# DOGECOIN87/firedancer

Measured on AMD Instinct MI355X. Metric: verified ed25519 sigs/sec (node), higher is better.
Workload: dtype u32; 1 GPU; cfg2: 1000000 single-sig txns/GPU, msg U[180,220] B, 90% valid / 10% corrupted, device-resident batch, full verify + per-txn combine per step; parallelism=dp1 (independent per-GPU batches), queues=2

## Files before the change

firedancer_amd/_lib.py:

```python
import ctypes
import os

_HERE = os.path.dirname(os.path.abspath(__file__))
LIB_PATH = os.environ.get("FDGPU_LIB") or os.path.join(_HERE, "libfd_ed25519_gpu.so")
HEADER_PATH = os.path.join(os.path.dirname(_HERE), "include", "fd_ed25519_gpu.h")
SHRED_HEADER_PATH = os.path.join(os.path.dirname(_HERE), "include", "fd_shred_gpu.h")
POH_HEADER_PATH = os.path.join(os.path.dirname(_HERE), "include", "fd_poh_gpu.h")

_LIB = None


class FdgpuTxn(ctypes.Structure):
    _fields_ = [("msg_off", ctypes.c_uint32), ("msg_sz", ctypes.c_uint32),
                ("sig_off", ctypes.c_uint32), ("pub_off", ctypes.c_uint32),
                ("sig_cnt", ctypes.c_uint32)]


class FdgpuCfg(ctypes.Structure):
    _fields_ = [("max_txn", ctypes.c_uint64), ("max_sig", ctypes.c_uint64),
                ("max_arena", ctypes.c_uint64), ("ring_depth", ctypes.c_uint32),
                ("flags", ctypes.c_uint32)]


def lib():
    global _LIB
    if _LIB is not None:
        return _LIB
    if not os.path.exists(LIB_PATH):
        raise RuntimeError(f"firedancer_amd: engine library not built: {LIB_PATH} "
                           "(run `make -C firedancer_amd/csrc`)")
    L = ctypes.CDLL(LIB_PATH)
    c = ctypes
    vp, u8p = c.c_void_p, c.c_char_p
    L.fd_ed25519_verify.argtypes = [u8p, c.c_uint64, u8p, u8p, vp]
    L.fd_ed25519_verify.restype = c.c_int
    L.fd_ed25519_verify_batch_single_msg.argtypes = [u8p, c.c_uint64, u8p, u8p, vp, c.c_uint8]
    L.fd_ed25519_verify_batch_single_msg.restype = c.c_int
    L.fd_ed25519_strerror.argtypes = [c.c_int]
    L.fd_ed25519_strerror.restype = c.c_char_p
    L.fdgpu_engine_open.argtypes = [c.c_int, c.POINTER(FdgpuCfg)]
    L.fdgpu_engine_open.restype = vp
    L.fdgpu_engine_reserve.argtypes = [vp, c.c_uint64]
    L.fdgpu_engine_reserve.restype = c.c_int
    L.fdgpu_engine_close.argtypes = [vp]
    L.fdgpu_engine_close.restype = None
    L.fdgpu_last_error.argtypes = []
    L.fdgpu_last_error.restype = c.c_char_p
    L.fdgpu_device_count.argtypes = []
    L.fdgpu_device_count.restype = c.c_int
    L.fdgpu_kernel_path.argtypes = []
    L.fdgpu_kernel_path.restype = c.c_char_p
    L.fdgpu_build_info.argtypes = []
    L.fdgpu_build_info.restype = c.c_char_p
    L.fdgpu_submit.argtypes = [vp, vp, c.c_uint64, vp, c.c_uint64]
    L.fdgpu_submit.restype = c.c_int64
    L.fdgpu_poll.argtypes = [vp, c.c_int64, vp, c.c_int]
    L.fdgpu_poll.restype = c.c_int
    L.fdgpu_stage_acquire.argtypes = [vp, c.POINTER(c.c_uint64)]
    L.fdgpu_stage_acquire.restype = vp
    L.fdgpu_stage_submit.argtypes = [vp, c.c_uint64, vp, c.c_uint64]
    L.fdgpu_stage_submit.restype = c.c_int64
    L.fdgpu_poll_keep.argtypes = [vp, c.c_int64, vp, c.c_int]
    L.fdgpu_poll_keep.restype = c.c_int
    L.fdgpu_release.argtypes = [vp, c.c_int64]
    L.fdgpu_release.restype = c.c_int
    L.fdgpu_stage_cancel.argtypes = [vp]
    L.fdgpu_stage_cancel.restype = c.c_int
    L.fdgpu_host_register.argtypes = [vp, vp, c.c_uint64]
    L.fdgpu_host_register.restype = c.c_int
    L.fdgpu_host_unregister.argtypes = [vp, vp]
    L.fdgpu_host_unregister.restype = c.c_int
    L.fdgpu_verify_device.argtypes = [vp, vp, vp, c.c_uint64, vp, c.c_uint64, vp, vp, vp]
    L.fdgpu_verify_device.restype = c.c_int
    L.fdgpu_engine_info.argtypes = [vp, c.POINTER(c.c_uint32), c.POINTER(c.c_uint32), c.POINTER(c.c_uint64)]
    L.fdgpu_engine_info.restype = c.c_int
    L.fdgpu_debug_fe_ops.argtypes = [vp, vp, c.c_uint64, vp]
    L.fdgpu_debug_decode.argtypes = [vp, vp, c.c_uint64, c.c_int, vp]
    L.fdgpu_debug_sha512.argtypes = [vp, vp, c.c_uint64, vp, c.c_uint64, vp]
    L.fdgpu_debug_hram.argtypes = [vp, vp, c.c_uint64, vp, c.c_uint64, vp]
    L.fdgpu_debug_sc_reduce.argtypes = [vp, vp, c.c_uint64, vp]
    L.fdgpu_debug_hs_split.argtypes = [vp, vp, c.c_uint64, vp]
    L.fdgpu_debug_sig_codes.argtypes = [vp, vp, c.c_uint64, vp, c.c_uint64, vp]
    L.fdgpu_dev_batch_upload.argtypes = [vp, vp, c.c_uint64, vp, c.c_uint64]
    L.fdgpu_dev_batch_upload.restype = vp
    L.fdgpu_dev_batch_verify.argtypes = [vp, vp]
    L.fdgpu_dev_batch_verify.restype = c.c_int
    L.fdgpu_dev_batch_own_queue.argtypes = [vp, vp]
    L.fdgpu_dev_batch_own_queue.restype = c.c_int
    L.fdgpu_dev_batch_codes.argtypes = [vp, vp, vp, vp]
    L.fdgpu_dev_batch_codes.restype = c.c_int
    L.fdgpu_dev_batch_upload_frags.argtypes = [vp, vp, c.c_uint64, vp, c.c_uint64]
    L.fdgpu_dev_batch_upload_frags.restype = vp
    L.fdgpu_dev_batch_txns.argtypes = [vp, vp, vp, vp]
    L.fdgpu_dev_batch_txns.restype = c.c_int
    L.fdgpu_dev_batch_time2.argtypes = [vp, vp, c.c_int] + [c.POINTER(c.c_double)] * 4
    L.fdgpu_dev_batch_time2.restype = c.c_int
    L.fdgpu_dev_batch_free.argtypes = [vp, vp]
    L.fdgpu_dev_batch_free.restype = None
    L.fdgpu_dev_batch_sig_cnt.argtypes = [vp]
    L.fdgpu_dev_batch_sig_cnt.restype = c.c_uint64
    L.fdgpu_dev_batch_device_ptrs.argtypes = [vp] + [vp] * 6
    L.fdgpu_dev_batch_device_ptrs.restype = c.c_int
    L.fdgpu_dev_batch_time.argtypes = [vp, vp, c.c_int, c.POINTER(c.c_double), c.POINTER(c.c_double),
                                       c.POINTER(c.c_double)]
    L.fdgpu_dev_batch_time.restype = c.c_int
    L.fdgpu_sync.argtypes = [vp]
    L.fdgpu_sync.restype = c.c_int
    L.fdgpu_submit_frags.argtypes = [vp, vp, c.c_uint64, vp, c.c_uint64, c.c_uint64]
    L.fdgpu_submit_frags.restype = c.c_int64
    L.fdgpu_poll_frags.argtypes = [vp, c.c_int64, vp, vp, c.c_int]
    L.fdgpu_poll_frags.restype = c.c_int
    L.fdgpu_submit_frags_io.argtypes = [vp, vp, c.c_uint64, vp, c.c_uint64, c.c_uint64, vp, c.c_uint64]
    L.fdgpu_submit_frags_io.restype = c.c_int64
    L.fdgpu_poll_frags_io.argtypes = [vp, c.c_int64, vp, vp, vp, c.c_int]
    L.fdgpu_poll_frags_io.restype = c.c_int
    L.fdgpu_debug_submit_times.argtypes = [vp, c.c_uint64]
    L.fdgpu_debug_submit_times.restype = c.c_uint64
    L.fdgpu_debug_h2d_gbps.argtypes = [vp, vp, c.c_uint64, c.c_int]
    L.fdgpu_debug_h2d_gbps.restype = c.c_double
    L.fdgpu_frag_out_cap.argtypes = [c.c_uint32]
    L.fdgpu_frag_out_cap.restype = c.c_uint32
    L.fdgpu_ed25519_verify.argtypes = [u8p, c.c_uint64, u8p, u8p]
    L.fdgpu_ed25519_verify.restype = c.c_int
    L.fdgpu_ed25519_verify_batch_single_msg.argtypes = [u8p, c.c_uint64, u8p, u8p, c.c_uint8]
    L.fdgpu_ed25519_verify_batch_single_msg.restype = c.c_int
    L.fdgpu_sync_stats.argtypes = [c.POINTER(c.c_uint64)] * 3
    L.fdgpu_sync_stats.restype = None
    L.fdgpu_sync_errors.argtypes = []
    L.fdgpu_sync_errors.restype = c.c_uint64
    L.fdgpu_submit_shreds.argtypes = [vp, vp, c.c_uint64, vp, c.c_uint64, c.c_uint16]
    L.fdgpu_submit_shreds.restype = c.c_int64
    L.fdgpu_poll_shreds.argtypes = [vp, c.c_int64, vp, vp, c.c_int]
    L.fdgpu_poll_shreds.restype = c.c_int
    L.fdgpu_debug_sha256.argtypes = [vp, vp, c.c_uint64, vp, c.c_uint64, vp]
    L.fdgpu_debug_sha256.restype = c.c_int
    L.fdgpu_debug_shred_roots.argtypes = [vp, vp, c.c_uint64, vp, c.c_uint64, c.c_uint16, vp, vp]
    L.fdgpu_debug_shred_roots.restype = c.c_int
    L.fdgpu_debug_shred_time.argtypes = [vp, vp, c.c_uint64, vp, c.c_uint64, c.c_uint16, c.c_int,
                                         c.POINTER(c.c_double), c.POINTER(c.c_double)]
    L.fdgpu_debug_shred_time.restype = c.c_int
    L.fdgpu_submit_poh.argtypes = [vp, vp, c.c_uint64, vp, c.c_uint64, vp, c.c_uint64, c.c_uint64]
    L.fdgpu_submit_poh.restype = c.c_int64
    L.fdgpu_poll_poh.argtypes = [vp, c.c_int64, vp, vp, c.c_int]
    L.fdgpu_poll_poh.restype = c.c_int
    L.fdgpu_poh_limits.argtypes = [vp] + [c.POINTER(c.c_uint64)] * 3
    L.fdgpu_poh_limits.restype = c.c_int
    L.fdgpu_poh_chunk.argtypes = []
    L.fdgpu_poh_chunk.restype = c.c_uint32
    L.fdgpu_debug_poh.argtypes = [vp, vp, c.c_uint64, vp, c.c_uint64, vp, c.c_uint64, c.c_uint64, c.c_uint32, vp, vp]
    L.fdgpu_debug_poh.restype = c.c_int
    L.fdgpu_debug_poh_time.argtypes = [vp, vp, c.c_uint64, vp, c.c_uint64, vp, c.c_uint64, c.c_uint64, c.c_int,
                                       c.POINTER(c.c_double), c.POINTER(c.c_double)]
    L.fdgpu_debug_poh_time.restype = c.c_int
    L.fdgpu_debug_fe_raw.argtypes = [vp, vp, c.c_uint64, vp]
    L.fdgpu_debug_ge_ops.argtypes = [vp, vp, c.c_uint64, vp]
    L.fdgpu_debug_sc_recode.argtypes = [vp, vp, c.c_uint64, vp]
    L.fdgpu_debug_btab.argtypes = [vp, c.c_uint64, c.c_uint64, vp]
    L.fdgpu_bcomb_dim.argtypes = [c.c_int]
    L.fdgpu_bcomb_dim.restype = c.c_uint32
    L.fdgpu_test_ge_in_words.argtypes = []
    L.fdgpu_test_ge_in_words.restype = c.c_uint32
    L.fdgpu_test_ge_results.argtypes = []
    L.fdgpu_test_ge_results.restype = c.c_uint32
    for fn in ("fdgpu_debug_fe_ops", "fdgpu_debug_decode", "fdgpu_debug_sha512", "fdgpu_debug_hram",
               "fdgpu_debug_sc_reduce", "fdgpu_debug_hs_split", "fdgpu_debug_sig_codes",
               "fdgpu_debug_fe_raw", "fdgpu_debug_ge_ops", "fdgpu_debug_sc_recode", "fdgpu_debug_btab"):
        getattr(L, fn).restype = c.c_int
    _LIB = L
    return L


def header_functions(path=None):
    import re
    text = open(path or HEADER_PATH).read()
    text = re.sub(r"/\*.*?\*/", "", text, flags=re.S)
    names = re.findall(r"^[A-Za-z_][\w \t\*]*?\b(fd\w+)\s*\(", text, flags=re.M)
    return sorted(set(n for n in names if not n.startswith("FD_")))


def build_info():
    import json
    return json.loads(lib().fdgpu_build_info().decode())


def require_product_build(allow_ab=False):
    info = build_info()
    if not info.get("product") and not allow_ab:
        raise RuntimeError(f"firedancer_amd: {LIB_PATH} is not the product build: {info} "
                           "(rebuild with `make -C firedancer_amd/csrc`, or pass the A/B flag)")
    return info


def last_error():
    return lib().fdgpu_last_error().decode()
```

firedancer_amd/csrc/fdgpu_diag.cpp:

```cpp
#include "fdgpu_engine.h"

using namespace fdgpu;

#define DALLOC(buf, n) do { if ((buf).alloc((size_t)(n) * sizeof(*(buf).p) + 64) != hipSuccess) { \
  set_err("alloc"); return FDGPU_ERR_DEVICE; } } while (0)

static int debug_msgs(fdgpu_engine_t *e, uint8_t const *arena, uint64_t arena_sz, fdgpu_txn_t const *txns, uint64_t n,
                      uint8_t *out, int hram) {
  if (!e || !n) return FDGPU_ERR_INVAL;
  HIPCHK(hipSetDevice(e->device), FDGPU_ERR_DEVICE);
  std::vector<fdgpu_sig_desc_t> d(n);
  for (uint64_t i = 0; i < n; i++) {
    if ((uint64_t)txns[i].msg_off + txns[i].msg_sz > arena_sz ||
        (hram && ((uint64_t)txns[i].sig_off + 64 > arena_sz || (uint64_t)txns[i].pub_off + 32 > arena_sz))) {
      set_err("descriptor out of bounds"); return FDGPU_ERR_INVAL;
    }
    d[i].msg_off = txns[i].msg_off; d[i].msg_sz = txns[i].msg_sz;
    d[i].sig_off = txns[i].sig_off; d[i].pub_off = txns[i].pub_off;
  }
  DevBuf<uint8_t> da;
  DevBuf<fdgpu_sig_desc_t> dd;
  DevBuf<uint32_t> dout;
  DALLOC(da, arena_sz + FDGPU_ARENA_SLACK);
  DALLOC(dd, n);
  DALLOC(dout, n * 16);
  HIPCHK(hipMemset(da, 0, arena_sz + FDGPU_ARENA_SLACK), FDGPU_ERR_DEVICE);
  if (arena_sz) HIPCHK(hipMemcpy(da, arena, arena_sz, hipMemcpyHostToDevice), FDGPU_ERR_DEVICE);
  HIPCHK(hipMemcpy(dd, d.data(), n * sizeof(fdgpu_sig_desc_t), hipMemcpyHostToDevice), FDGPU_ERR_DEVICE);
  if (hram)
    HIPCHK(fdgpu_launch_test_hram(da, dd, (uint32_t)n, dout, e->compute), FDGPU_ERR_DEVICE);
  else
    HIPCHK(fdgpu_launch_test_sha512(da, dd, (uint32_t)n, dout, e->compute), FDGPU_ERR_DEVICE);
  HIPCHK(hipStreamSynchronize(e->compute), FDGPU_ERR_DEVICE);
  HIPCHK(hipMemcpy(out, dout, n * (hram ? 32 : 64), hipMemcpyDeviceToHost), FDGPU_ERR_DEVICE);
  return FDGPU_OK;
}

template <class Launch>
static int debug_map(fdgpu_engine_t *e, uint8_t const *in, uint64_t n, uint64_t in_words, uint64_t out_words,
                     uint8_t *out, Launch launch) {
  if (!e || !n) return FDGPU_ERR_INVAL;
  HIPCHK(hipSetDevice(e->device), FDGPU_ERR_DEVICE);
  DevBuf<uint32_t> din, dout;
  DALLOC(din, n * in_words);
  DALLOC(dout, n * out_words);
  HIPCHK(hipMemcpy(din, in, n * in_words * 4, hipMemcpyHostToDevice), FDGPU_ERR_DEVICE);
  HIPCHK(launch(din.p, dout.p, (uint32_t)n, e->compute), FDGPU_ERR_DEVICE);
  HIPCHK(hipStreamSynchronize(e->compute), FDGPU_ERR_DEVICE);
  HIPCHK(hipMemcpy(out, dout, n * out_words * 4, hipMemcpyDeviceToHost), FDGPU_ERR_DEVICE);
  return FDGPU_OK;
}

extern "C" {

int fdgpu_debug_fe_ops(fdgpu_engine_t *e, uint8_t const *ab, uint64_t n, uint8_t *out) {
  return debug_map(e, ab, n, 16, 64, out, fdgpu_launch_test_fe);
}

int fdgpu_debug_decode(fdgpu_engine_t *e, uint8_t const *enc, uint64_t n, int ref_mapping, uint8_t *out) {
  const uint32_t flags = ref_mapping ? FDGPU_FLAG_REF_MAP : 0u;
  return debug_map(e, enc, n, 8, 18, out, [flags](const uint32_t *i, uint32_t *o, uint32_t k, hipStream_t st) {
    return fdgpu_launch_test_decode(i, o, k, flags, st);
  });
}

int fdgpu_debug_sha512(fdgpu_engine_t *e, uint8_t const *arena, uint64_t arena_sz, fdgpu_txn_t const *msgs,
                       uint64_t n, uint8_t *out) {
  return debug_msgs(e, arena, arena_sz, msgs, n, out, 0);
}

int fdgpu_debug_hram(fdgpu_engine_t *e, uint8_t const *arena, uint64_t arena_sz, fdgpu_txn_t const *txns,
                     uint64_t n, uint8_t *out) {
  return debug_msgs(e, arena, arena_sz, txns, n, out, 1);
}

int fdgpu_debug_sc_reduce(fdgpu_engine_t *e, uint8_t const *in, uint64_t n, uint8_t *out) {
  return debug_map(e, in, n, 16, 8, out, fdgpu_launch_test_sc_reduce);
}

int fdgpu_debug_hs_split(fdgpu_engine_t *e, uint8_t const *k, uint64_t n, uint8_t *out) {
  return debug_map(e, k, n, 8, 16, out, fdgpu_launch_test_hs_split);
}

int fdgpu_debug_fe_raw(fdgpu_engine_t *e, uint8_t const *fg, uint64_t n, uint8_t *out) {
  return debug_map(e, fg, n, 20, 80, out, fdgpu_launch_test_fe_raw);
}

int fdgpu_debug_ge_ops(fdgpu_engine_t *e, uint8_t const *in, uint64_t n, uint8_t *out) {
  return debug_map(e, in, n, fdgpu_test_ge_in_words(), 32u * fdgpu_test_ge_results(), out, fdgpu_launch_test_ge);
}

int fdgpu_debug_sc_recode(fdgpu_engine_t *e, uint8_t const *s, uint64_t n, uint8_t *out) {
  return debug_map(e, s, n, 8, 16, out, fdgpu_launch_test_sc_recode);
}

int fdgpu_debug_btab(fdgpu_engine_t *e, uint64_t first_entry, uint64_t n_entries, uint32_t *out) {
  const uint64_t total = (uint64_t)FDGPU_BCOMB_NDIG * FDGPU_BCOMB_ENTRIES;
  if (!e || !e->d_btab || !out || first_entry > total || n_entries > total - first_entry) {
    set_err("fdgpu_debug_btab: entries out of the table"); return FDGPU_ERR_INVAL;
  }
  if (!n_entries) return FDGPU_OK;
  HIPCHK(hipSetDevice(e->device), FDGPU_ERR_DEVICE);
  HIPCHK(hipStreamSynchronize(e->compute), FDGPU_ERR_DEVICE);
  HIPCHK(hipMemcpy(out, e->d_btab + first_entry * FDGPU_BCOMB_STRIDE, n_entries * FDGPU_BCOMB_STRIDE * sizeof(uint32_t),
                   hipMemcpyDeviceToHost), FDGPU_ERR_DEVICE);
  return FDGPU_OK;
}

uint32_t fdgpu_bcomb_dim(int which) {
  switch (which) {
    case 0: return FDGPU_BCOMB_BITS;
    case 1: return FDGPU_BCOMB_NDIG;
    case 2: return FDGPU_BCOMB_ENTRIES;
    case 3: return FDGPU_BCOMB_STRIDE;
    case 4: return FDGPU_BCOMB_CHUNK;
    default: return 0u;
  }
}

int fdgpu_debug_sig_codes(fdgpu_engine_t *e, uint8_t const *arena, uint64_t arena_sz, fdgpu_txn_t const *txns,
                          uint64_t txn_cnt, int8_t *sig_codes) {
  if (!e) return FDGPU_ERR_INVAL;
  HIPCHK(hipSetDevice(e->device), FDGPU_ERR_DEVICE);
  uint64_t total = 0;
  for (uint64_t t = 0; t < txn_cnt; t++) total += (txns[t].sig_cnt >= 1 && txns[t].sig_cnt <= 16) ? txns[t].sig_cnt : 0;
  std::vector<fdgpu_sig_desc_t> sd(total + 1);
  std::vector<fdgpu_txn_desc_t> td(txn_cnt + 1);
  std::vector<uint32_t> pm(total + 1);
  uint32_t *perm = bucket(e) ? pm.data() : nullptr;
  const int64_t ns = expand(arena_sz, txns, txn_cnt, total, sd.data(), td.data(), perm);
  if (ns < 0) return FDGPU_ERR_INVAL;
  if (!ns) return FDGPU_OK;
  DevBuf<uint8_t> da;
  DevBuf<fdgpu_sig_desc_t> dd;
  DevBuf<uint32_t> dp;
  DevBuf<int8_t> dc;
  DALLOC(da, arena_sz + FDGPU_ARENA_SLACK);
  DALLOC(dd, ns);
  DALLOC(dp, ns);
  DALLOC(dc, ns);
  HIPCHK(hipMemset(da, 0, arena_sz + FDGPU_ARENA_SLACK), FDGPU_ERR_DEVICE);
  HIPCHK(hipMemcpy(da, arena, arena_sz, hipMemcpyHostToDevice), FDGPU_ERR_DEVICE);
  HIPCHK(hipMemcpy(dd, sd.data(), ns * sizeof(fdgpu_sig_desc_t), hipMemcpyHostToDevice), FDGPU_ERR_DEVICE);
  if (perm) HIPCHK(hipMemcpy(dp, perm, ns * sizeof(uint32_t), hipMemcpyHostToDevice), FDGPU_ERR_DEVICE);
  const uint32_t flags = kflags(e);
  if ((uint64_t)ns > e->ws_sig) { int rc = ensure_ws(e, (uint64_t)ns); if (rc) return rc; }
  HIPCHK(fdgpu_launch_verify_sigs(da, dd, (uint32_t)ns, perm ? dp.p : nullptr, e->d_btab, e->d_ws, dc, flags,
                                  e->compute, nullptr, e->resident_blocks, e->kc_seed),
         FDGPU_ERR_DEVICE);
  HIPCHK(hipStreamSynchronize(e->compute), FDGPU_ERR_DEVICE);
  HIPCHK(hipMemcpy(sig_codes, dc, ns, hipMemcpyDeviceToHost), FDGPU_ERR_DEVICE);
  return FDGPU_OK;
}

}
```

firedancer_amd/csrc/fdgpu_internal.h:

```cpp
#pragma once

#include <hip/hip_runtime_api.h>
#include <stddef.h>
#include <stdint.h>

#include "../../include/fd_ed25519_gpu.h"
#include "../../include/fd_poh_gpu.h"

typedef struct {
  uint32_t msg_off;
  uint32_t msg_sz;
  uint32_t sig_off;
  uint32_t pub_off;
} fdgpu_sig_desc_t;

typedef struct {
  uint32_t sig0;
  uint32_t sig_cnt;
} fdgpu_txn_desc_t;

#define FDGPU_ARENA_SLACK   160u
#define FDGPU_ATAB_ENTRIES  9u
#ifndef FDGPU_ATAB_WORDS
#define FDGPU_ATAB_WORDS    40u
#endif
#ifndef FDGPU_VERIFY_WAVES
#define FDGPU_VERIFY_WAVES  2
#endif
#ifndef FDGPU_PHASE_STAMPS
#define FDGPU_PHASE_STAMPS  0
#endif
#define FDGPU_BCOMB_BITS    16u
#define FDGPU_BCOMB_NDIG    ((254u + FDGPU_BCOMB_BITS - 1u) / FDGPU_BCOMB_BITS)
#define FDGPU_BCOMB_ENTRIES ((1u << (FDGPU_BCOMB_BITS - 1u)) + 1u)
#define FDGPU_BCOMB_STRIDE  32u
#define FDGPU_BCOMB_CHUNK   64u
#define HS_MAX_WIN          40u
#define FDGPU_TAB_STORED    (FDGPU_ATAB_ENTRIES - 1u)
#define FDGPU_WS_RTAB       FDGPU_TAB_STORED
#define FDGPU_WS_PARK       (2u * FDGPU_TAB_STORED)
#define FDGPU_WS_SB         (FDGPU_WS_PARK + 1u)
#define FDGPU_WS_ENTRIES    (FDGPU_WS_SB + 1u)
#define FDGPU_WS_LANE_WORDS (FDGPU_WS_ENTRIES * FDGPU_ATAB_WORDS)
#define FDGPU_BLOCK         256u
#define FDGPU_FLAG_REF_MAP  1u
#define FDGPU_FLAG_KFULL    2u
#define FDGPU_FLAG_KCACHE   4u
#define FDGPU_FLAG_KPAIR    8u
#define FDGPU_FLAG_KSPREAD  16u
#define FDGPU_SPREAD_LDS       1024u
#define FDGPU_SPREAD_LDS_PAIR  (40u * 1024u + 1024u)
#define FDGPU_FULL_BLOCKS   16u
#define FDGPU_AUX_BLOCKS    64u
#define FDGPU_IO_BLOCKS     16u
#define FDGPU_NBLK_GROUPS   32u
#define FDGPU_POH_CHUNK     64u

#ifdef __cplusplus
extern "C" {
#endif


size_t     fdgpu_btab_bytes(void);
hipError_t fdgpu_btab_build(uint32_t *d_btab, hipStream_t stream);

hipError_t fdgpu_launch_verify_sigs(const uint8_t *d_arena, const fdgpu_sig_desc_t *d_sigs, uint32_t n_sig,
                                    const uint32_t *d_perm, const uint32_t *d_btab, uint32_t *d_ws,
                                    int8_t *d_sig_codes, uint32_t flags, hipStream_t stream,
                                    const uint32_t *d_n_sig, uint32_t resident_blocks, uint64_t kc_seed,
                                    int cnt_zeroed = 0);
uint64_t   fdgpu_sha512_stream_blocks(uint64_t msg_sz);
hipError_t fdgpu_launch_sha512_stream(const uint8_t *d_mbuf, uint64_t m0, uint64_t mlen, uint64_t msg_sz,
                                      uint64_t blk0, uint32_t nblk, const uint8_t *d_ra, uint64_t *d_state,
                                      uint32_t n, hipStream_t stream);
hipError_t fdgpu_launch_verify_prehashed(const uint8_t *d_arena, const fdgpu_sig_desc_t *d_sigs, uint32_t n_sig,
                                         const uint32_t *d_btab, uint32_t *d_ws, int8_t *d_sig_codes, uint32_t flags,
                                         hipStream_t stream);
typedef struct {
  uint64_t lanes, ht_slots;
  uint32_t *queue, *cnt, *rep_cnt, *ht, *key_of, *kverd, *reps;
  size_t bytes;
} fdgpu_ws_layout_t;
static inline fdgpu_ws_layout_t fdgpu_ws_layout(uint32_t *d_ws, uint64_t n_sig) {
  fdgpu_ws_layout_t l;
  l.lanes = (n_sig + FDGPU_BLOCK - 1) / FDGPU_BLOCK * FDGPU_BLOCK;
  for (l.ht_slots = 64; l.ht_slots < 2 * l.lanes;) l.ht_slots <<= 1;
  const uint64_t queue = l.lanes * FDGPU_WS_LANE_WORDS, cnt = queue + l.lanes, ht = cnt + 16, key_of = ht + l.ht_slots;
  auto at = [d_ws](uint64_t word) { return d_ws ? d_ws + word : nullptr; };
  l.queue = at(queue);
  l.cnt = at(cnt);
  l.rep_cnt = at(cnt + 1);
  l.ht = at(ht);
  l.key_of = at(key_of);
  l.kverd = at(key_of + l.lanes);
  l.reps = at(key_of + 2 * l.lanes);
  l.bytes = (size_t)(key_of + 3 * l.lanes) * sizeof(uint32_t);
  return l;
}
typedef struct {
  const uint8_t *arena;
  const fdgpu_sig_desc_t *sigs;
  const uint32_t *n_sig;
  uint32_t *ws;
  int8_t *codes;
  uint32_t *queue, *cnt;
  uint32_t bound;
  uint32_t slow;
} fdgpu_mbatch_t;
hipError_t fdgpu_launch_verify_multi(const fdgpu_mbatch_t *mb, uint32_t nb, uint32_t grid_max, uint32_t slow_max,
                                     const uint32_t *d_btab, uint32_t flags, hipStream_t stream);
hipError_t fdgpu_launch_combine(const fdgpu_txn_desc_t *d_txns, uint32_t n_txn, const int8_t *d_sig_codes,
                                int8_t *d_txn_codes, uint64_t *d_accept, hipStream_t stream);
hipError_t fdgpu_verify_occupancy(int *blocks_per_cu);
int        fdgpu_kernel_build_info(char *buf, size_t n);
size_t     fdgpu_ws_bytes(uint64_t n_sig);

__attribute__((visibility("hidden"))) hipError_t fdgpu_ingest_load(void);
uint64_t   fdgpu_frag_sig_bound(uint32_t sz);
hipError_t fdgpu_launch_frag_ingest(const uint8_t *d_arena, const void *d_frags, uint32_t frag_stride, uint32_t n,
                                    uint8_t *d_txn_out, uint16_t *d_txn_sz, fdgpu_txn_t *d_txd, uint32_t *d_cnt,
                                    uint32_t *d_sig0, uint32_t *d_blocktot, uint32_t *d_n_sig,
                                    fdgpu_sig_desc_t *d_sigs, fdgpu_txn_desc_t *d_tds, hipStream_t stream);
hipError_t fdgpu_launch_frag_codes(const uint16_t *d_txn_sz, uint32_t n, int8_t *d_codes, hipStream_t stream);
#define FDGPU_SMALL_SCAN_MAX 65536u
hipError_t fdgpu_launch_frag_ring(const uint8_t *d_arena, const fdgpu_frag_ex_t *d_fx, uint32_t n, uint8_t *d_txn_out,
                                  uint16_t *d_txn_sz, fdgpu_txn_t *d_txd, uint32_t *d_cnt, uint32_t *d_sig0,
                                  uint32_t *d_blocktot, uint32_t *d_n_sig, fdgpu_sig_desc_t *d_sigs,
                                  fdgpu_txn_desc_t *d_tds, hipStream_t stream);
hipError_t fdgpu_launch_frag_finish(const fdgpu_txn_desc_t *d_tds, uint32_t n, const int8_t *d_sig_codes,
                                    const uint16_t *d_txn_sz, const fdgpu_frag_ex_t *d_fx, const uint8_t *d_txn_out,
                                    int8_t *d_codes, uint8_t *d_trailers, hipStream_t stream);
#define FDGPU_FX_LAPPED 0x80000000u
#define FDGPU_IO_RANGES_MAX 255u
uint64_t   fdgpu_frag_fp_bound(uint32_t sz);
hipError_t fdgpu_launch_frag_ingest_io(const uint64_t *d_src, const fdgpu_frag_ex_t *d_fx, const uint64_t *d_chk,
                                       const uint64_t *d_rtab, uint32_t n, uint8_t *d_arena,
                                       fdgpu_frag_ex_t *d_fx_dev, uint8_t *d_txn_out, uint16_t *d_txn_sz,
                                       fdgpu_sig_desc_t *d_sigs, fdgpu_txn_desc_t *d_tds, uint32_t *d_n_sig,
                                       uint32_t *d_zero_word, hipStream_t stream);
hipError_t fdgpu_launch_frag_finish_io(const fdgpu_txn_desc_t *d_tds, uint32_t n, const int8_t *d_sig_codes,
                                       const uint16_t *d_txn_sz, const fdgpu_frag_ex_t *d_fx, const uint8_t *d_txn_out,
                                       const uint8_t *d_arena, uint64_t hash_seed, uint8_t *d_out, int8_t *d_codes,
                                       uint64_t *d_tags, uint16_t *d_out_szs, uint32_t *d_zero_next,
                                       hipStream_t stream);

hipError_t fdgpu_launch_poh_tree(const uint8_t *d_arena, const fdgpu_poh_entry_t *d_entries, uint32_t n,
                                 const uint32_t *d_sig_offs, uint32_t sig_total, uint32_t *d_nodes, hipStream_t stream);
hipError_t fdgpu_launch_poh_chains(const uint8_t *d_arena, const fdgpu_poh_entry_t *d_entries, uint32_t n,
                                   const uint32_t *d_order, uint32_t n_q, const uint32_t *d_nodes, uint32_t cap,
                                   uint32_t grid_waves, uint32_t *d_head, int8_t *d_codes, uint8_t *d_hashes,
                                   hipStream_t stream);

hipError_t fdgpu_launch_test_fe(const uint32_t *d_in, uint32_t *d_out, uint32_t n, hipStream_t stream);
hipError_t fdgpu_launch_test_decode(const uint32_t *d_enc, uint32_t *d_out, uint32_t n, uint32_t flags, hipStream_t stream);
hipError_t fdgpu_launch_test_sha512(const uint8_t *d_arena, const fdgpu_sig_desc_t *d_msgs, uint32_t n,
                                    uint32_t *d_out, hipStream_t stream);
hipError_t fdgpu_launch_test_hram(const uint8_t *d_arena, const fdgpu_sig_desc_t *d_sigs, uint32_t n,
                                  uint32_t *d_out, hipStream_t stream);
hipError_t fdgpu_launch_test_sc_reduce(const uint32_t *d_in, uint32_t *d_out, uint32_t n, hipStream_t stream);
hipError_t fdgpu_launch_test_hs_split(const uint32_t *d_in, uint32_t *d_out, uint32_t n, hipStream_t stream);
hipError_t fdgpu_launch_test_fe_raw(const uint32_t *d_in, uint32_t *d_out, uint32_t n, hipStream_t stream);
uint32_t   fdgpu_test_ge_in_words(void);
uint32_t   fdgpu_test_ge_results(void);
hipError_t fdgpu_launch_test_ge(const uint32_t *d_in, uint32_t *d_out, uint32_t n, hipStream_t stream);
hipError_t fdgpu_launch_test_sc_recode(const uint32_t *d_in, uint32_t *d_out, uint32_t n, hipStream_t stream);

int      fdgpu_debug_fe_raw(fdgpu_engine_t *e, uint8_t const *fg, uint64_t n, uint8_t *out);
int      fdgpu_debug_ge_ops(fdgpu_engine_t *e, uint8_t const *in, uint64_t n, uint8_t *out);
int      fdgpu_debug_sc_recode(fdgpu_engine_t *e, uint8_t const *s, uint64_t n, uint8_t *out);
int      fdgpu_debug_btab(fdgpu_engine_t *e, uint64_t first_entry, uint64_t n_entries, uint32_t *out);
uint32_t fdgpu_bcomb_dim(int which);

#ifdef __cplusplus
}
#endif
```

firedancer_amd/csrc/fdgpu_test_kernels.hip:

```cpp
#include <hip/hip_runtime.h>

#include "fdgpu_ge.h"
#include "fdgpu_hram.h"
#include "fdgpu_internal.h"
#include "fdgpu_lattice.h"
#include "fdgpu_sc.h"
#include "fdgpu_sha512.h"

using namespace fdgpu;

namespace {

__global__ void __launch_bounds__(64) fdgpu_test_fe_kernel(const uint32_t *in, uint32_t *out, uint32_t n) {
  const uint32_t i = blockIdx.x * blockDim.x + threadIdx.x;
  if (i >= n) return;
  uint32_t aw[8], bw[8];
#pragma unroll
  for (int j = 0; j < 8; j++) { aw[j] = in[16 * i + j]; bw[j] = in[16 * i + 8 + j]; }
  fe a, b, r;
  fe_frombytes(a, aw); fe_frombytes(b, bw);
  uint32_t o[8];
  uint32_t *dst = out + 64 * i;
  fe_mul(r, a, b); fe_tobytes(o, r);
  for (int j = 0; j < 8; j++) dst[j] = o[j];
  fe_sq(r, a); fe_tobytes(o, r);
  for (int j = 0; j < 8; j++) dst[8 + j] = o[j];
  fe_add(r, a, b); fe_tobytes(o, r);
  for (int j = 0; j < 8; j++) dst[16 + j] = o[j];
  fe_sub(r, a, b); fe_tobytes(o, r);
  for (int j = 0; j < 8; j++) dst[24 + j] = o[j];
  fe_pow22523(r, a); fe_tobytes(o, r);
  for (int j = 0; j < 8; j++) dst[32 + j] = o[j];
  fe_invert(r, a); fe_tobytes(o, r);
  for (int j = 0; j < 8; j++) dst[40 + j] = o[j];
  fe_tobytes(o, a);
  for (int j = 0; j < 8; j++) dst[48 + j] = o[j];
  fe_neg(r, a); fe_tobytes(o, r);
  for (int j = 0; j < 8; j++) dst[56 + j] = o[j];
}

__global__ void __launch_bounds__(64) fdgpu_test_decode_kernel(const uint32_t *enc, uint32_t *out, uint32_t n, uint32_t flags) {
  const uint32_t i = blockIdx.x * blockDim.x + threadIdx.x;
  if (i >= n) return;
  uint32_t e[8];
  for (int j = 0; j < 8; j++) e[j] = enc[8 * i + j];
  ge_p3 P;
  const bool ok = ge_decode(P, e, (flags & FDGPU_FLAG_REF_MAP) != 0);
  uint32_t *dst = out + 18 * i;
  dst[0] = ok ? 0u : 0xffffffffu;
  dst[1] = ok ? (ge_is_small_order_affine(P) ? 1u : 0u) : 0xffffffffu;
  uint32_t x[8], y[8];
  fe_tobytes(x, P.X); fe_tobytes(y, P.Y);
  for (int j = 0; j < 8; j++) { dst[2 + j] = x[j]; dst[10 + j] = y[j]; }
}

__global__ void __launch_bounds__(64) fdgpu_test_sha512_kernel(const uint8_t *arena, const fdgpu_sig_desc_t *msgs, uint32_t n,
                                         uint32_t *out) {
  const uint32_t i = blockIdx.x * blockDim.x + threadIdx.x;
  const bool active = i < n;
  const fdgpu_sig_desc_t d = msgs[active ? i : n - 1];
  uint32_t nb = (d.msg_sz + 16u) / 128u + 1u;
  for (int off = 32; off > 0; off >>= 1) nb = max(nb, (uint32_t)__shfl_xor((int)nb, off));
  uint64_t h[8];
  sha512_plain(h, arena + d.msg_off, d.msg_sz, nb);
  if (!active) return;
  for (int j = 0; j < 8; j++) {
    out[16 * i + 2 * j] = bswap32((uint32_t)(h[j] >> 32));
    out[16 * i + 2 * j + 1] = bswap32((uint32_t)h[j]);
  }
}

__global__ void __launch_bounds__(64) fdgpu_test_hram_kernel(const uint8_t *arena, const fdgpu_sig_desc_t *sigs, uint32_t n,
                                       uint32_t *out) {
  const uint32_t i = blockIdx.x * blockDim.x + threadIdx.x;
  const bool active = i < n;
  const fdgpu_sig_desc_t d = sigs[active ? i : n - 1];
  const uint32_t nb = wave_max_u32(sha512_hram_blocks(d.msg_sz));
  uint32_t R[8], A[8], k[8];
  load32(R, arena + d.sig_off);
  load32(A, arena + d.pub_off);
  hram_k(k, R, A, arena, d, nb);
  if (!active) return;
  for (int j = 0; j < 8; j++) out[8 * i + j] = k[j];
}

__global__ void __launch_bounds__(64) fdgpu_test_sc_reduce_kernel(const uint32_t *in, uint32_t *out, uint32_t n) {
  const uint32_t i = blockIdx.x * blockDim.x + threadIdx.x;
  if (i >= n) return;
  uint32_t x[16], r[8];
  for (int j = 0; j < 16; j++) x[j] = in[16 * i + j];
  sc_reduce512(r, x);
  for (int j = 0; j < 8; j++) out[8 * i + j] = r[j];
}

__global__ void __launch_bounds__(64) fdgpu_test_hs_split_kernel(const uint32_t *in, uint32_t *out, uint32_t n) {
  const uint32_t i = blockIdx.x * blockDim.x + threadIdx.x;
  uint32_t k[8];
  for (int j = 0; j < 8; j++) k[j] = i < n ? in[8 * i + j] : 0u;
  hs_split_t o;
  hs_split(o, k);
  if (i >= n) return;
  uint32_t *w = out + 16 * (size_t)i;
  for (int j = 0; j < 5; j++) { w[j] = o.u[j]; w[5 + j] = o.v[j]; }
  w[10] = o.ok; w[11] = o.u_neg; w[12] = o.v_neg; w[13] = o.bits; w[14] = 0u; w[15] = 0u;
}

FDG_DEV void put_fe(uint32_t *dst, const fe &f) {
  uint32_t o[8];
  fe_tobytes(o, f);
#pragma unroll
  for (int j = 0; j < 8; j++) dst[j] = o[j];
}

__global__ void __launch_bounds__(64) fdgpu_test_fe_raw_kernel(const uint32_t *in, uint32_t *out, uint32_t n) {
  const uint32_t i = blockIdx.x * blockDim.x + threadIdx.x;
  if (i >= n) return;
  fe f, g, r, s;
#pragma unroll
  for (int j = 0; j < 10; j++) { f.v[j] = in[20 * (size_t)i + j]; g.v[j] = in[20 * (size_t)i + 10 + j]; }
  uint32_t *dst = out + 80 * (size_t)i;
  fe_mul(r, f, g);  put_fe(dst, r);
  fe_sq(r, f);      put_fe(dst + 8, r);
  fe_add(r, f, g);  put_fe(dst + 16, r);
  fe_sub(s, f, g);  put_fe(dst + 24, s);
  fe_mul(r, s, g);  put_fe(dst + 32, r);
  fe_neg(s, f);     put_fe(dst + 40, s);
  fe_mul(r, s, g);  put_fe(dst + 48, r);
  put_fe(dst + 56, f);
  fe_sub4(s, f, g); put_fe(dst + 64, s);
  fe_mul(r, s, g);  put_fe(dst + 72, r);
}

FDG_DEV void get_fe(fe &h, const uint32_t *src) {
  uint32_t w[8];
#pragma unroll
  for (int j = 0; j < 8; j++) w[j] = src[j];
  fe_frombytes(h, w);
}
FDG_DEV void put_p3(uint32_t *dst, const ge_p3 &p) {
  put_fe(dst, p.X); put_fe(dst + 8, p.Y); put_fe(dst + 16, p.Z); put_fe(dst + 24, p.T);
}
FDG_DEV void put_p2(uint32_t *dst, const ge_p2 &p) {
  put_fe(dst, p.X); put_fe(dst + 8, p.Y); put_fe(dst + 16, p.Z);
#pragma unroll
  for (int j = 0; j < 8; j++) dst[24 + j] = 0u;
}
FDG_DEV void put_p1p1(uint32_t *dst, const ge_p1p1 &t) {
  ge_p3 r;
  ge_p1p1_to_p3(r, t);
  put_p3(dst, r);
}

#define GE_IN_WORDS  88u
#define GE_RESULTS   21u
#define GE_OUT_WORDS (GE_RESULTS * 32u)

__global__ void __launch_bounds__(64) fdgpu_test_ge_kernel(const uint32_t *in, uint32_t *out, uint32_t n) {
  const uint32_t i = blockIdx.x * blockDim.x + threadIdx.x;
  if (i >= n) return;
  const uint32_t *src = in + GE_IN_WORDS * (size_t)i;
  uint32_t *dst = out + GE_OUT_WORDS * (size_t)i;
  ge_p3 P, Q;
  get_fe(P.X, src); get_fe(P.Y, src + 8); get_fe(P.Z, src + 16); get_fe(P.T, src + 24);
  get_fe(Q.X, src + 32); get_fe(Q.Y, src + 40); get_fe(Q.Z, src + 48); get_fe(Q.T, src + 56);
  ge_niels N;
  get_fe(N.ypx, src + 64); get_fe(N.ymx, src + 72); get_fe(N.xy2d, src + 80);
  ge_cached C;
  ge_p3_to_cached(C, Q);
  uint32_t qc[40], qn[32];
#pragma unroll
  for (int w = 0; w < 10; w++) {
    qc[w] = C.YpX.v[w]; qc[10 + w] = C.YmX.v[w]; qc[20 + w] = C.Z2.v[w]; qc[30 + w] = C.T2d.v[w];
    qn[w] = N.ypx.v[w]; qn[10 + w] = N.ymx.v[w]; qn[20 + w] = N.xy2d.v[w];
  }
  qn[30] = 0u; qn[31] = 0u;

  ge_p1p1 t;
  ge_p2 a2;
  ge_p3 r3;
  ge_p3_to_p2(a2, P);
  ge_dbl(t, a2);
  put_p1p1(dst, t);
  ge_p1p1_to_p2(a2, t);
  put_p2(dst + 32, a2);

  auto ldc = [&C](int c, int w) { return c == 0 ? C.YpX.v[w] : c == 1 ? C.YmX.v[w] : c == 2 ? C.Z2.v[w] : C.T2d.v[w]; };
#pragma unroll 1
  for (int s = 0; s < 2; s++) {
    const bool neg = s != 0;
    uint32_t *d = dst + 32 * s;
    ge_add_cached(t, P, C, neg);          put_p1p1(d + 32 * 2, t);
    ge_add_cached_ld(t, P, ldc, neg);     put_p1p1(d + 32 * 4, t);
    ge_add_cached_regs(t, P, qc, neg);    put_p1p1(d + 32 * 6, t);
    uint32_t qs[40];
#pragma unroll
    for (int w = 0; w < 10; w++) {
      qs[w] = neg ? qc[10 + w] : qc[w]; qs[10 + w] = neg ? qc[w] : qc[10 + w]; qs[20 + w] = qc[20 + w]; qs[30 + w] = qc[30 + w];
    }
    ge_add_cached_regs_swapped(t, P, qs, neg); put_p1p1(d + 32 * 8, t);
    ge_add_niels(t, P, N, neg);           put_p1p1(d + 32 * 10, t);
    ge_add_niels_regs(t, P, qn, neg);     put_p1p1(d + 32 * 12, t);
    ge_cached_regs_to_p2(a2, qc, neg);    put_p2(d + 32 * 14, a2);
    ge_niels_regs_to_p3(r3, qn, neg);     put_p3(d + 32 * 16, r3);

    ge_p3_to_p2(a2, P);
#pragma unroll 1
    for (int k = 0; k < 4; k++) { ge_dbl(t, a2); ge_p1p1_to_p2(a2, t); }
    r3.X = a2.X; r3.Y = a2.Y; r3.Z = a2.Z; fe_mul(r3.T, t.X, t.Y);
    ge_add_cached_regs_swapped(t, r3, qc, false);
    ge_p1p1_to_p3(r3, t);
    ge_add_cached_regs_swapped(t, r3, qs, neg);
    put_p1p1(d + 32 * 19, t);
  }
  ge_p3_neg(r3, P);
  put_p3(dst + 32 * 18, r3);
}

__global__ void __launch_bounds__(64) fdgpu_test_sc_recode_kernel(const uint32_t *in, uint32_t *out, uint32_t n) {
  const uint32_t i = blockIdx.x * blockDim.x + threadIdx.x;
  if (i >= n) return;
  constexpr int NW = COMB_WORDS(FDGPU_BCOMB_BITS, FDGPU_BCOMB_NDIG);
  static_assert(NW <= 8, "the record holds 8 words of comb digits");
  uint32_t s[8], d16[8], dc[NW];
  for (int j = 0; j < 8; j++) s[j] = in[8 * (size_t)i + j];
  sc_recode16(d16, s);
  sc_recode_comb<(int)FDGPU_BCOMB_BITS, (int)FDGPU_BCOMB_NDIG>(dc, s);
  uint32_t *w = out + 16 * (size_t)i;
  for (int j = 0; j < 8; j++) { w[j] = d16[j]; w[8 + j] = j < NW ? dc[j] : 0u; }
}

}

extern "C" {

hipError_t fdgpu_launch_test_fe(const uint32_t *d_in, uint32_t *d_out, uint32_t n, hipStream_t stream) {
  hipLaunchKernelGGL(fdgpu_test_fe_kernel, dim3((n + 63) / 64), dim3(64), 0, stream, d_in, d_out, n);
  return hipGetLastError();
}
hipError_t fdgpu_launch_test_decode(const uint32_t *d_enc, uint32_t *d_out, uint32_t n, uint32_t flags,
                                    hipStream_t stream) {
  hipLaunchKernelGGL(fdgpu_test_decode_kernel, dim3((n + 63) / 64), dim3(64), 0, stream, d_enc, d_out, n, flags);
  return hipGetLastError();
}
hipError_t fdgpu_launch_test_sha512(const uint8_t *d_arena, const fdgpu_sig_desc_t *d_msgs, uint32_t n,
                                    uint32_t *d_out, hipStream_t stream) {
  hipLaunchKernelGGL(fdgpu_test_sha512_kernel, dim3((n + 63) / 64), dim3(64), 0, stream, d_arena, d_msgs, n, d_out);
  return hipGetLastError();
}
hipError_t fdgpu_launch_test_hram(const uint8_t *d_arena, const fdgpu_sig_desc_t *d_sigs, uint32_t n,
                                  uint32_t *d_out, hipStream_t stream) {
  hipLaunchKernelGGL(fdgpu_test_hram_kernel, dim3((n + 63) / 64), dim3(64), 0, stream, d_arena, d_sigs, n, d_out);
  return hipGetLastError();
}
hipError_t fdgpu_launch_test_sc_reduce(const uint32_t *d_in, uint32_t *d_out, uint32_t n, hipStream_t stream) {
  hipLaunchKernelGGL(fdgpu_test_sc_reduce_kernel, dim3((n + 63) / 64), dim3(64), 0, stream, d_in, d_out, n);
  return hipGetLastError();
}
hipError_t fdgpu_launch_test_hs_split(const uint32_t *d_in, uint32_t *d_out, uint32_t n, hipStream_t stream) {
  hipLaunchKernelGGL(fdgpu_test_hs_split_kernel, dim3((n + 63) / 64), dim3(64), 0, stream, d_in, d_out, n);
  return hipGetLastError();
}
hipError_t fdgpu_launch_test_fe_raw(const uint32_t *d_in, uint32_t *d_out, uint32_t n, hipStream_t stream) {
  hipLaunchKernelGGL(fdgpu_test_fe_raw_kernel, dim3((n + 63) / 64), dim3(64), 0, stream, d_in, d_out, n);
  return hipGetLastError();
}
uint32_t fdgpu_test_ge_in_words(void) { return GE_IN_WORDS; }
uint32_t fdgpu_test_ge_results(void) { return GE_RESULTS; }
hipError_t fdgpu_launch_test_ge(const uint32_t *d_in, uint32_t *d_out, uint32_t n, hipStream_t stream) {
  hipLaunchKernelGGL(fdgpu_test_ge_kernel, dim3((n + 63) / 64), dim3(64), 0, stream, d_in, d_out, n);
  return hipGetLastError();
}
hipError_t fdgpu_launch_test_sc_recode(const uint32_t *d_in, uint32_t *d_out, uint32_t n, hipStream_t stream) {
  hipLaunchKernelGGL(fdgpu_test_sc_recode_kernel, dim3((n + 63) / 64), dim3(64), 0, stream, d_in, d_out, n);
  return hipGetLastError();
}

}
```

firedancer_amd/csrc/fdgpu_verify.hip:

```cpp
#include <hip/hip_runtime.h>

#include "fdgpu_bcomb.h"
#include "fdgpu_ge.h"
#include "fdgpu_hram.h"
#include "fdgpu_internal.h"
#include "fdgpu_lattice.h"
#include "fdgpu_sc.h"
#include "fdgpu_sha512.h"
#include "fdgpu_stamps.h"

using namespace fdgpu;

namespace {


__host__ __device__ constexpr int atab_pos(int w) {
  return w >= 20 ? w : w < 10 ? 4 * (w / 2) + (w % 2) : 4 * ((w - 10) / 2) + 2 + (w % 2);
}

struct alignas(16) tab_ident_t { uint32_t w[FDGPU_ATAB_WORDS]; };
__device__ const tab_ident_t g_tab_ident = {{1u, 0u, 1u, 0u, 0u, 0u, 0u, 0u, 0u, 0u, 0u, 0u, 0u, 0u, 0u, 0u, 0u, 0u, 0u, 0u, 2u}};
static_assert(atab_pos(0) == 0 && atab_pos(10) == 2 && atab_pos(20) == 20, "identity entry's stored order");

FDG_DEV const uint32_t *tab_entry(const uint32_t *tab, int e) {
  return e ? tab + (uint32_t)(e < 0 ? -e : e) * FDGPU_ATAB_WORDS : g_tab_ident.w;
}
FDG_DEV uint32_t *tab_a(uint32_t *wsl) { return wsl - FDGPU_ATAB_WORDS; }
FDG_DEV const uint32_t *tab_a(const uint32_t *wsl) { return wsl - FDGPU_ATAB_WORDS; }
FDG_DEV uint32_t *tab_r(uint32_t *wsl) { return wsl + (FDGPU_WS_RTAB - 1u) * FDGPU_ATAB_WORDS; }

FDG_DEV void atab_store(uint32_t *wsl, uint32_t entry, const ge_cached &c) {
  uint4 *p = (uint4 *)(wsl + entry * FDGPU_ATAB_WORDS);
  uint32_t w[40], o[40];
#pragma unroll
  for (int i = 0; i < 10; i++) { w[i] = c.YpX.v[i]; w[10 + i] = c.YmX.v[i]; w[20 + i] = c.Z2.v[i]; w[30 + i] = c.T2d.v[i]; }
#pragma unroll
  for (int i = 0; i < 40; i++) o[atab_pos(i)] = w[i];
#pragma unroll
  for (int q = 0; q < 10; q++) p[q] = make_uint4(o[4 * q], o[4 * q + 1], o[4 * q + 2], o[4 * q + 3]);
}
FDG_DEV int sext4(uint32_t x) { return ((int)(x << 28)) >> 28; }

#define KD_WORDS 8

FDG_DEV void atab_load(uint32_t (&q)[40], const uint32_t *wsl, int e) {
  const uint4 *ent = (const uint4 *)tab_entry(wsl, e);
  uint32_t o[40];
#pragma unroll
  for (int i = 0; i < 10; i++) {
    const uint4 v = ent[i];
    o[4 * i] = v.x; o[4 * i + 1] = v.y; o[4 * i + 2] = v.z; o[4 * i + 3] = v.w;
  }
#pragma unroll
  for (int i = 0; i < 40; i++) q[i] = o[atab_pos(i)];
}

FDG_DEV void shl4(uint32_t (&w)[8]) {
#pragma unroll
  for (int i = 7; i > 0; i--) w[i] = (w[i] << 4) | (w[i - 1] >> 28);
  w[0] <<= 4;
}

FDG_DEV void dsm_k(ge_p2 &acc2, uint32_t (&kd)[KD_WORDS], const uint32_t *wsl, uint32_t sb_entry = FDGPU_WS_SB,
                   const uint32_t *ta = nullptr) {
  if (!ta) ta = tab_a(wsl);
  ge_p3 acc3;
  ge_p1p1 t;
  uint32_t q[40];
  {
    const int e = sext4(kd[7] >> 28);
    shl4(kd);
    atab_load(q, ta, e);
    ge_cached_regs_to_p2(acc2, q, e < 0);
  }
#pragma unroll 1
  for (int j = 62; j >= 0; j--) {
    const int e = sext4(kd[7] >> 28);
    shl4(kd);
    atab_load(q, ta, e);
#pragma unroll 1
    for (int r = 0; r < 4; r++) {
      ge_dbl(t, acc2);
      ge_p1p1_to_p2(acc2, t);
    }
    acc3.X = acc2.X; acc3.Y = acc2.Y; acc3.Z = acc2.Z; fe_mul(acc3.T, t.X, t.Y);
    ge_add_cached_regs(t, acc3, q, e < 0);
    if (j == 0) break;
    ge_p1p1_to_p2(acc2, t);
  }
  ge_p1p1_to_p3(acc3, t);
  uint32_t qs[40];
  atab_load(qs, wsl, (int)sb_entry);
  ge_add_cached_regs(t, acc3, qs, false);
  ge_p1p1_to_p2(acc2, t);
}

FDG_DEV void comb_sb(ge_p3 &acc, const uint32_t (&S)[8], const uint32_t *__restrict__ btab, uint32_t lo = 0,
                     uint32_t hi = BC_NDIG) {
  constexpr int NW = COMB_WORDS(BC_W, BC_NDIG), SLOT = COMB_SLOT(BC_W);
  uint32_t dg[NW];
  sc_recode_comb<(int)BC_W, (int)BC_NDIG>(dg, S);
  auto next_digit = [&dg]() {
    const int d = SLOT == 16 ? (int)(int16_t)(dg[0] & 0xffffu) : (int)dg[0];
#pragma unroll
    for (int i = 0; i < NW - 1; i++) dg[i] = SLOT == 16 ? (dg[i] >> 16) | (dg[i + 1] << 16) : dg[i + 1];
    dg[NW - 1] = SLOT == 16 ? dg[NW - 1] >> 16 : 0u;
    return d;
  };
  auto load_entry = [btab](uint32_t (&q)[32], uint32_t ti, int d) {
    const uint4 *ent = (const uint4 *)(btab + ((size_t)ti * BC_ENT + (uint32_t)(d < 0 ? -d : d)) * FDGPU_BCOMB_STRIDE);
#pragma unroll
    for (int i = 0; i < 8; i++) {
      const uint4 v = ent[i];
      q[4 * i] = v.x; q[4 * i + 1] = v.y; q[4 * i + 2] = v.z; q[4 * i + 3] = v.w;
    }
  };
  uint32_t qa[32], qb[32];
#pragma unroll 1
  for (uint32_t i = 0; i < lo; i++) (void)next_digit();
  int d = next_digit();
  load_entry(qa, lo, d);
  {
    const int dn = next_digit();
    load_entry(qb, lo + 1, dn);
    ge_niels_regs_to_p3(acc, qa, d < 0);
#pragma unroll
    for (int w = 0; w < 32; w++) qa[w] = qb[w];
    d = dn;
  }
  ge_p1p1 t;
#pragma unroll 1
  for (uint32_t i = lo + 1; i < hi; i++) {
    const int dn = next_digit();
    if (i + 1 < hi) load_entry(qb, i + 1, dn);
    ge_add_niels_regs(t, acc, qa, d < 0);
    ge_p1p1_to_p3(acc, t);
#pragma unroll
    for (int w = 0; w < 32; w++) qa[w] = qb[w];
    d = dn;
  }
}

FDG_DEV void atab_build(uint32_t *wsl, const ge_p3 &An) {
  ge_cached c;
  ge_p3_to_cached(c, An); atab_store(wsl, 1, c);
  ge_p1p1 t; ge_p2 a2; ge_p3 P;
  ge_p3_to_p2(a2, An); ge_dbl(t, a2); ge_p1p1_to_p3(P, t);
  ge_p3_to_cached(c, P); atab_store(wsl, 2, c);
  const uint32_t *ent1 = wsl + 1u * FDGPU_ATAB_WORDS;
  auto ld1 = [ent1](int cc, int w) { return ent1[atab_pos(10 * cc + w)]; };
#pragma unroll 1
  for (uint32_t e = 3; e < FDGPU_ATAB_ENTRIES; e++) {
    if (e & 1u) {
      ge_add_cached_ld(t, P, ld1, false);
    } else {
      uint32_t q[40];
      atab_load(q, wsl, (int)(e >> 1));
      ge_cached_regs_to_p2(a2, q, false);
      ge_dbl(t, a2);
    }
    ge_p1p1_to_p3(P, t);
    ge_p3_to_cached(c, P); atab_store(wsl, e, c);
  }
}

FDG_DEV uint32_t *lane_ws(uint32_t *ws, uint32_t i) {
  return ws + (size_t)i * FDGPU_WS_LANE_WORDS;
}

FDG_DEV uint32_t out_idx(const uint32_t *__restrict__ perm, uint32_t i) { return perm ? perm[i] : i; }


#define HPARK_KD 0
#define HPARK_CODE 30
static_assert(HPARK_KD + KD_WORDS <= HPARK_CODE && HPARK_CODE < (int)FDGPU_ATAB_WORDS, "park layout");

FDG_DEV void recode16_160(uint32_t (&out)[5], uint32_t &nd, const uint32_t (&m)[5]) {
  uint32_t carry = 0;
  nd = 0;
#pragma unroll
  for (int w = 0; w < 5; w++) {
    uint32_t o = 0;
#pragma unroll
    for (int n = 0; n < 8; n++) {
      uint32_t e = ((m[w] >> (4 * n)) & 15u) + carry;
      carry = e >= 8u;
      e = (e - (carry << 4)) & 15u;
      o |= e << (4 * n);
      nd = e ? (uint32_t)(8 * w + n + 1) : nd;
    }
    out[w] = o;
  }
  nd = carry ? 41u : nd;
}

FDG_DEV void shl4_5(uint32_t (&w)[5]) {
#pragma unroll
  for (int i = 4; i > 0; i--) w[i] = (w[i] << 4) | (w[i - 1] >> 28);
  w[0] <<= 4;
}

FDG_DEV void hs_wscalar(uint32_t (&w)[8], const uint32_t (&v)[5], bool v_neg, const uint32_t (&S)[8]) {
  uint32_t x[16];
#pragma unroll
  for (int i = 0; i < 16; i++) x[i] = 0;
#pragma unroll
  for (int i = 0; i < 5; i++) {
    uint64_t c = 0;
#pragma unroll
    for (int j = 0; j < 8; j++) {
      const uint64_t t = (uint64_t)v[i] * S[j] + x[i + j] + c;
      x[i + j] = (uint32_t)t;
      c = t >> 32;
    }
    x[i + 8] = (uint32_t)c;
  }
  uint32_t r[8];
  sc_reduce512(r, x);
  constexpr uint32_t L[8] = FDGPU_SC_L;
  uint32_t nz = 0;
#pragma unroll
  for (int i = 0; i < 8; i++) nz |= r[i];
  const bool flip = v_neg && nz != 0;
  uint32_t bw = 0;
#pragma unroll
  for (int i = 0; i < 8; i++) {
    const uint64_t d = (uint64_t)L[i] - r[i] - bw;
    w[i] = flip ? (uint32_t)d : r[i];
    bw = (uint32_t)(d >> 63);
  }
}

typedef __attribute__((address_space(3))) void lds_void_t;

FDG_DEV void stage_entry(uint32_t *lds_wave, const uint32_t *tab, int e) {
  const uint32_t *src = tab_entry(tab, e);
  constexpr int NCH = 10;
#pragma unroll
  for (int c = 0; c < NCH; c++)
    __builtin_amdgcn_global_load_lds((const void *)(src + 4 * c), (lds_void_t *)(lds_wave + 256 * c), 16, 0, 0);
}

FDG_DEV void unstage_entry_signed(uint32_t (&q)[40], const uint32_t *lds_wave, bool neg) {
  const uint32_t lane = threadIdx.x & 63u;
  const uint32_t *a = lds_wave + 4 * lane + (neg ? 2u : 0u), *b = lds_wave + 4 * lane + (neg ? 0u : 2u);
#pragma unroll
  for (int c = 0; c < 5; c++) {
    const uint2 x = *(const uint2 *)(a + 256 * c), y = *(const uint2 *)(b + 256 * c);
    q[2 * c] = x.x; q[2 * c + 1] = x.y; q[10 + 2 * c] = y.x; q[10 + 2 * c + 1] = y.y;
  }
#pragma unroll
  for (int c = 5; c < 10; c++) {
    const uint4 v = *(const uint4 *)(lds_wave + 256 * c + 4 * lane);
    q[4 * c] = v.x; q[4 * c + 1] = v.y; q[4 * c + 2] = v.z; q[4 * c + 3] = v.w;
  }
}

FDG_DEV void hs_chain(ge_p1p1 &t, uint32_t (&ud)[5], uint32_t (&vd)[5], bool u_neg, bool v_neg, uint32_t nwin,
                      const uint32_t *wsl, const uint32_t *ta) {
  const uint32_t *tr = tab_r(const_cast<uint32_t *>(wsl));
  __shared__ uint32_t s_stage[FDGPU_BLOCK / 64][2][10 * 256];
  uint32_t *st_r = &s_stage[threadIdx.x >> 6][0][0];
  uint32_t *st_a = &s_stage[threadIdx.x >> 6][1][0];
  ge_p2 acc2;
  ge_p3 acc3;
  uint32_t q[40];
  {
    const int du = sext4(ud[4] >> 28), dv = sext4(vd[4] >> 28);
    shl4_5(ud); shl4_5(vd);
    atab_load(q, ta, du);
    ge_p3_0(acc3);
    ge_add_cached_regs(t, acc3, q, (du < 0) != u_neg);
    ge_p1p1_to_p3(acc3, t);
    atab_load(q, tr, dv);
    ge_add_cached_regs(t, acc3, q, (dv < 0) != v_neg);
  }
#pragma unroll 1
  for (uint32_t j = 1; j < nwin; j++) {
    ge_p1p1_to_p2(acc2, t);
    const int du = sext4(ud[4] >> 28), dv = sext4(vd[4] >> 28);
    shl4_5(ud); shl4_5(vd);
    stage_entry(st_a, ta, du);
    stage_entry(st_r, tr, dv);
#pragma unroll 1
    for (int r = 0; r < 4; r++) {
      ge_dbl(t, acc2);
      ge_p1p1_to_p2(acc2, t);
    }
    acc3.X = acc2.X; acc3.Y = acc2.Y; acc3.Z = acc2.Z; fe_mul(acc3.T, t.X, t.Y);
    asm volatile("s_waitcnt vmcnt(0)" ::: "memory");
    unstage_entry_signed(q, st_a, (du < 0) != u_neg);
    ge_add_cached_regs_swapped(t, acc3, q, (du < 0) != u_neg);
    ge_p1p1_to_p3(acc3, t);
    unstage_entry_signed(q, st_r, (dv < 0) != v_neg);
    ge_add_cached_regs_swapped(t, acc3, q, (dv < 0) != v_neg);
  }
}


FDG_DEV uint32_t decode_neg_table(uint32_t *tab, const uint32_t (&enc)[8], bool ref_map) {
  ge_p3 P, Pn;
  const bool ok = ge_decode(P, enc, ref_map);
  const bool small = ge_is_small_order_affine(P);
  ge_p3_neg(Pn, P);
  atab_build(tab, Pn);
  return (ok ? 1u : 0u) | (small ? 2u : 0u);
}

FDG_DEV void hs_split_masked(hs_split_t &hs, const uint32_t (&k)[8], bool need) {
  uint32_t ke[8];
#pragma unroll
  for (int j = 0; j < 8; j++) ke[j] = need ? k[j] : 0u;
  hs_split(hs, ke);
}

FDG_DEV uint32_t hs_digits(uint32_t (&ud)[5], uint32_t (&vd)[5], const hs_split_t &hs) {
  uint32_t ndu = 0, ndv = 0;
  recode16_160(ud, ndu, hs.u);
  recode16_160(vd, ndv, hs.v);
  return max(max(ndu, ndv), 1u);
}

FDG_DEV void comb_scalar(uint32_t (&w)[8], const hs_split_t &hs, const uint32_t (&S)[8], bool half) {
  hs_wscalar(w, hs.v, hs.v_neg, S);
#pragma unroll
  for (int j = 0; j < 8; j++) w[j] = half ? w[j] : S[j];
}

FDG_DEV void park_full(uint32_t *park, const uint32_t (&k)[8]) {
  uint32_t kd[KD_WORDS];
  sc_recode16(kd, k);
#pragma unroll
  for (int j = 0; j < KD_WORDS; j++) park[HPARK_KD + j] = kd[j];
  park[HPARK_CODE] = 0u;
}

FDG_DEV void queue_full_lanes(uint32_t *queue, uint32_t *queue_cnt, bool q_full, uint32_t i) {
  const uint64_t m = __ballot(q_full);
  if (m) {
    const int lane = (int)(threadIdx.x & 63u);
    const int leader = __ffsll((long long)m) - 1;
    uint32_t base = 0;
    if (lane == leader) base = atomicAdd(queue_cnt, (uint32_t)__popcll(m));
    base = (uint32_t)__shfl((int)base, leader, 64);
    if (q_full) queue[base + (uint32_t)__popcll(m & ((1ull << lane) - 1ull))] = i;
  }
}

template <bool KC, bool PH = false>
FDG_DEV void verify_hs_body(const uint8_t *__restrict__ arena, const fdgpu_sig_desc_t *__restrict__ sigs, uint32_t n_sig_arg,
                            const uint32_t *__restrict__ n_sig_dev, const uint32_t *__restrict__ btab,
                            uint32_t *__restrict__ ws, const uint32_t *__restrict__ perm, int8_t *__restrict__ codes,
                            uint32_t *__restrict__ queue, uint32_t *__restrict__ queue_cnt, uint32_t flags,
                            const uint32_t *__restrict__ key_of, const uint32_t *__restrict__ kverd, uint32_t bx) {
  const uint32_t n_sig = n_sig_dev ? *n_sig_dev : n_sig_arg;
  if (bx * blockDim.x >= n_sig) return;
  const uint32_t i = bx * blockDim.x + threadIdx.x;
  const bool active = i < n_sig;
  const bool ref_map = (flags & FDGPU_FLAG_REF_MAP) != 0;
  const fdgpu_sig_desc_t d = sigs[active ? i : n_sig - 1];
  uint32_t nb = sha512_hram_blocks(d.msg_sz);
#pragma unroll
  for (int off = 32; off > 0; off >>= 1) nb = max(nb, (uint32_t)__shfl_xor((int)nb, off));
  uint32_t *wsl = lane_ws(ws, i);
  uint32_t *park = wsl + FDGPU_WS_PARK * FDGPU_ATAB_WORDS;
  const uint32_t *ta = tab_a(wsl);
  FDGPU_STAMP(0);
  uint32_t Renc[8], Aenc[8];
  load32(Renc, arena + d.sig_off);
  load32(Aenc, arena + d.pub_off);
  uint32_t k[8];
  {
    uint64_t h[8];
    if (PH) {
#pragma unroll
      for (int j = 0; j < 8; j++) h[j] = ((const uint64_t *)(arena + d.msg_off))[j];
    } else {
      sha512_hram(h, Renc, Aenc, arena + d.msg_off, d.msg_sz, nb);
    }
    FDGPU_STAMP(1);
    uint32_t kx[16];
#pragma unroll
    for (int j = 0; j < 8; j++) { kx[2 * j] = bswap32((uint32_t)(h[j] >> 32)); kx[2 * j + 1] = bswap32((uint32_t)h[j]); }
    sc_reduce512(k, kx);
  }
  uint32_t S[8];
  load32(S, arena + d.sig_off + 32);
  int code = sc_lt_L(S) ? 0 : -1;
#pragma unroll
  for (int j = 0; j < 8; j++) S[j] = code ? 0u : S[j];
  FDGPU_STAMP(2);
  {
    ge_p3 P, Pn;
    bool a_ok, a_small;
    if (KC) {
      const uint32_t di = active ? i : n_sig - 1u, r = key_of[di], vd = kverd[r];
      a_ok = (vd & 1u) != 0;
      a_small = (vd & 2u) != 0;
      ta = tab_a(lane_ws(ws, r));
    } else {
      a_ok = ge_decode(P, Aenc, ref_map);
      a_small = ge_is_small_order_affine(P);
      ge_p3_neg(Pn, P);
      atab_build(tab_a(wsl), Pn);
    }
    FDGPU_STAMP(3);
    const bool r_ok = ge_decode(P, Renc, ref_map);
    const bool r_small = ge_is_small_order_affine(P);
    ge_p3_neg(Pn, P);
    atab_build(tab_r(wsl), Pn);
    if (code == 0 && !a_ok) code = ref_map ? -2 : -1;
    if (code == 0 && !r_ok) code = -1;
    if (code == 0 && a_small) code = -2;
    if (code == 0 && r_small) code = -1;
  }
  FDGPU_STAMP(4);
  const bool need = active && code == 0;
  hs_split_t hs;
  hs_split_masked(hs, k, need);
  uint32_t ud[5], vd[5];
  const uint32_t nd_lane = hs_digits(ud, vd, hs);
  const bool full = need && (!hs.ok || nd_lane > HS_MAX_WIN || (flags & FDGPU_FLAG_KFULL));
  const bool half = need && !full;
  FDGPU_STAMP(5);
  {
    uint32_t w[8];
    comb_scalar(w, hs, S, half);
    ge_p3 WB;
    comb_sb(WB, w, btab);
    ge_cached c; ge_p3_to_cached(c, WB);
    atab_store(wsl, FDGPU_WS_SB, c);
  }
  if (full) park_full(park, k);
  FDGPU_STAMP(6);
  bool eq = false;
  if (__any(half)) {
    const uint32_t nwin = wave_max_u32(half ? nd_lane : 1u);
#pragma unroll 1
    for (uint32_t s = nwin; s < 40; s++) { shl4_5(ud); shl4_5(vd); }
    ge_p1p1 t;
    hs_chain(t, ud, vd, hs.u_neg, hs.v_neg, nwin, wsl, ta);
    uint32_t q[40];
    atab_load(q, wsl, (int)FDGPU_WS_SB);
    fe ypx, ymx, z2, xw, yw, l1, l2;
#pragma unroll
    for (int j = 0; j < 10; j++) { ypx.v[j] = q[j]; ymx.v[j] = q[10 + j]; z2.v[j] = q[20 + j]; }
    fe_sub(xw, ypx, ymx);
    fe_add(yw, ypx, ymx);
    fe_mul(l1, t.X, z2);
    fe_mul(l2, t.Z, xw);
    fe_add(l1, l1, l2);
    const bool ex = fe_iszero(l1);
    fe_mul(l1, t.Y, z2);
    fe_mul(l2, t.T, yw);
    fe_sub(l1, l1, l2);
    eq = ex && fe_iszero(l1);
  }
  FDGPU_STAMP(7);
  if (active && !full) codes[out_idx(perm, i)] = (int8_t)(code ? code : (eq ? 0 : -3));
  queue_full_lanes(queue, queue_cnt, full, i);
}

template <bool KC, bool PH = false>
__global__ void __launch_bounds__(FDGPU_BLOCK, FDGPU_VERIFY_WAVES)
fdgpu_verify_hs_kernel(const uint8_t *__restrict__ arena, const fdgpu_sig_desc_t *__restrict__ sigs, uint32_t n_sig_arg,
                       const uint32_t *__restrict__ n_sig_dev, const uint32_t *__restrict__ btab,
                       uint32_t *__restrict__ ws, const uint32_t *__restrict__ perm, int8_t *__restrict__ codes,
                       uint32_t *__restrict__ queue, uint32_t *__restrict__ queue_cnt, uint32_t flags,
                       const uint32_t *__restrict__ key_of, const uint32_t *__restrict__ kverd) {
  verify_hs_body<KC, PH>(arena, sigs, n_sig_arg, n_sig_dev, btab, ws, perm, codes, queue, queue_cnt, flags, key_of,
                         kverd, blockIdx.x);
}

__global__ void __launch_bounds__(64) fdgpu_sha512_stream_kernel(const uint8_t *__restrict__ mbuf, uint64_t m0,
                                                                 uint64_t mlen, uint64_t msg_sz, uint64_t blk0,
                                                                 uint32_t nblk, const uint8_t *__restrict__ ra,
                                                                 uint64_t *__restrict__ state, uint32_t n) {
  const uint32_t i = threadIdx.x;
  if (i >= n) return;
  const uint64_t H0[8] = {0x6a09e667f3bcc908ULL, 0xbb67ae8584caa73bULL, 0x3c6ef372fe94f82bULL,
                          0xa54ff53a5f1d36f1ULL, 0x510e527fade682d1ULL, 0x9b05688c2b3e6c1fULL,
                          0x1f83d9abfb41bd6bULL, 0x5be0cd19137e2179ULL};
  uint64_t h[8];
  for (int j = 0; j < 8; j++) h[j] = blk0 ? state[8 * i + j] : H0[j];
  const uint64_t total = (64u + msg_sz + 16u) / 128u + 1u, bitlen = (64u + msg_sz) * 8u;
  for (uint64_t b = blk0; b < blk0 + nblk; b++) {
    uint64_t w[16];
    for (int t = 0; t < 16; t++) {
      uint64_t v = 0;
      for (int j = 0; j < 8; j++) {
        const uint64_t s = 128u * b + 8u * (uint64_t)t + (uint64_t)j;
        uint32_t byte;
        if (s < 64u) {
          byte = ra[64u * i + s];
        } else {
          const uint64_t g = s - 64u;
          byte = g < msg_sz ? (g >= m0 && g < m0 + mlen ? mbuf[g - m0] : 0u) : g == msg_sz ? 0x80u : 0u;
        }
        v = (v << 8) | byte;
      }
      w[t] = v;
    }
    if (b + 1 == total) { w[14] = 0; w[15] = bitlen; }
    sha512_compress(h, w);
  }
  for (int j = 0; j < 8; j++) state[8 * i + j] = h[j];
}

__global__ void __launch_bounds__(FDGPU_BLOCK, FDGPU_VERIFY_WAVES)
fdgpu_verify_hs_multi_kernel(const fdgpu_mbatch_t *__restrict__ mb, const uint32_t *__restrict__ btab, uint32_t flags) {
  const fdgpu_mbatch_t b = mb[blockIdx.y];
  if (blockIdx.x * blockDim.x >= b.bound) return;
  verify_hs_body<false>(b.arena, b.sigs, b.bound, b.n_sig, btab, b.ws, nullptr, b.codes, b.queue, b.cnt, flags, nullptr,
                        nullptr, blockIdx.x);
}


FDG_DEV void hs_chain1(ge_p1p1 &t, uint32_t (&dd)[5], bool neg, uint32_t nwin, const uint32_t *tab) {
  __shared__ uint32_t s_stage1[FDGPU_BLOCK / 64][10 * 256];
  uint32_t *st = &s_stage1[threadIdx.x >> 6][0];
  ge_p2 acc2;
  ge_p3 acc3;
  uint32_t q[40];
  {
    const int d = sext4(dd[4] >> 28);
    shl4_5(dd);
    atab_load(q, tab, d);
    ge_p3_0(acc3);
    ge_add_cached_regs(t, acc3, q, (d < 0) != neg);
  }
#pragma unroll 1
  for (uint32_t j = 1; j < nwin; j++) {
    ge_p1p1_to_p2(acc2, t);
    const int d = sext4(dd[4] >> 28);
    shl4_5(dd);
    stage_entry(st, tab, d);
#pragma unroll 1
    for (int r = 0; r < 4; r++) {
      ge_dbl(t, acc2);
      ge_p1p1_to_p2(acc2, t);
    }
    acc3.X = acc2.X; acc3.Y = acc2.Y; acc3.Z = acc2.Z; fe_mul(acc3.T, t.X, t.Y);
    asm volatile("s_waitcnt vmcnt(0)" ::: "memory");
    unstage_entry_signed(q, st, (d < 0) != neg);
    ge_add_cached_regs_swapped(t, acc3, q, (d < 0) != neg);
  }
}

FDG_DEV void fe_xchg_pair(fe &r, const fe &a) {
#pragma unroll
  for (int j = 0; j < 10; j++) r.v[j] = (uint32_t)__shfl_xor((int)a.v[j], 1);
}

__global__ void __launch_bounds__(FDGPU_BLOCK, FDGPU_VERIFY_WAVES)
fdgpu_verify_pair_kernel(const uint8_t *__restrict__ arena, const fdgpu_sig_desc_t *__restrict__ sigs, uint32_t n_sig_arg,
                         const uint32_t *__restrict__ n_sig_dev, const uint32_t *__restrict__ btab,
                         uint32_t *__restrict__ ws, const uint32_t *__restrict__ perm, int8_t *__restrict__ codes,
                         uint32_t *__restrict__ queue, uint32_t *__restrict__ queue_cnt, uint32_t flags) {
  const uint32_t n_sig = n_sig_dev ? *n_sig_dev : n_sig_arg;
  if (blockIdx.x * (blockDim.x / 2u) >= n_sig) return;
  const uint32_t g = blockIdx.x * blockDim.x + threadIdx.x, i = g >> 1;
  const bool rl = (g & 1u) != 0;
  const bool active = i < n_sig;
  const bool ref_map = (flags & FDGPU_FLAG_REF_MAP) != 0;
  const fdgpu_sig_desc_t d = sigs[active ? i : n_sig - 1];
  const uint32_t nb = wave_max_u32(sha512_hram_blocks(d.msg_sz));
  uint32_t *wsl = lane_ws(ws, i);
  uint32_t *tab = rl ? tab_r(wsl) : tab_a(wsl);
  uint32_t Renc[8], Aenc[8];
  load32(Renc, arena + d.sig_off);
  load32(Aenc, arena + d.pub_off);
  uint32_t k[8];
  hram_k(k, Renc, Aenc, arena, d, nb);
  uint32_t S[8];
  load32(S, arena + d.sig_off + 32);
  int code = sc_lt_L(S) ? 0 : -1;
#pragma unroll
  for (int j = 0; j < 8; j++) S[j] = code ? 0u : S[j];
  {
    uint32_t enc[8];
#pragma unroll
    for (int j = 0; j < 8; j++) enc[j] = rl ? Renc[j] : Aenc[j];
    const uint32_t mine = decode_neg_table(tab, enc, ref_map);
    const uint32_t other = (uint32_t)__shfl_xor((int)mine, 1);
    const uint32_t av = rl ? other : mine, rv = rl ? mine : other;
    if (code == 0 && !(av & 1u)) code = ref_map ? -2 : -1;
    if (code == 0 && !(rv & 1u)) code = -1;
    if (code == 0 && (av & 2u)) code = -2;
    if (code == 0 && (rv & 2u)) code = -1;
  }
  const bool need = active && code == 0;
  hs_split_t hs;
  hs_split_masked(hs, k, need);
  uint32_t ud[5], vd[5];
  const uint32_t nd_lane = hs_digits(ud, vd, hs);
  const bool full = need && (!hs.ok || nd_lane > HS_MAX_WIN || (flags & FDGPU_FLAG_KFULL));
  const bool half = need && !full;
  {
    uint32_t w[8];
    comb_scalar(w, hs, S, half);
    ge_p3 WB, WBo;
    comb_sb(WB, w, btab, rl ? BC_NDIG / 2u : 0u, rl ? BC_NDIG : BC_NDIG / 2u);
    fe_xchg_pair(WBo.X, WB.X);
    fe_xchg_pair(WBo.Y, WB.Y);
    fe_xchg_pair(WBo.Z, WB.Z);
    fe_xchg_pair(WBo.T, WB.T);
    ge_cached c; ge_p3_to_cached(c, WBo);
    ge_p1p1 tw; ge_add_cached(tw, WB, c, false);
    ge_p1p1_to_p3(WB, tw);
    ge_p3_to_cached(c, WB);
    if (!rl) atab_store(wsl, FDGPU_WS_SB, c);
  }
  if (full && !rl) park_full(wsl + FDGPU_WS_PARK * FDGPU_ATAB_WORDS, k);
  bool eq = false;
  if (__any(half)) {
    const uint32_t nwin = wave_max_u32(half ? nd_lane : 1u);
    uint32_t dd[5];
#pragma unroll
    for (int j = 0; j < 5; j++) dd[j] = rl ? vd[j] : ud[j];
#pragma unroll 1
    for (uint32_t s2 = nwin; s2 < 40; s2++) shl4_5(dd);
    ge_p1p1 t;
    hs_chain1(t, dd, rl ? hs.v_neg : hs.u_neg, nwin, tab);
    ge_p3 mine, other;
    ge_p1p1_to_p3(mine, t);
    fe_xchg_pair(other.X, mine.X);
    fe_xchg_pair(other.Y, mine.Y);
    fe_xchg_pair(other.Z, mine.Z);
    fe_xchg_pair(other.T, mine.T);
    ge_cached oc;
    ge_p3_to_cached(oc, other);
    ge_add_cached(t, mine, oc, false);
    uint32_t q[40];
    atab_load(q, wsl, (int)FDGPU_WS_SB);
    fe ypx, ymx, z2, xw, yw, l1, l2;
#pragma unroll
    for (int j = 0; j < 10; j++) { ypx.v[j] = q[j]; ymx.v[j] = q[10 + j]; z2.v[j] = q[20 + j]; }
    fe_sub(xw, ypx, ymx);
    fe_add(yw, ypx, ymx);
    fe_mul(l1, t.X, z2);
    fe_mul(l2, t.Z, xw);
    fe_add(l1, l1, l2);
    const bool ex = fe_iszero(l1);
    fe_mul(l1, t.Y, z2);
    fe_mul(l2, t.T, yw);
    fe_sub(l1, l1, l2);
    eq = ex && fe_iszero(l1);
  }
  if (active && !full && !rl) codes[out_idx(perm, i)] = (int8_t)(code ? code : (eq ? 0 : -3));
  queue_full_lanes(queue, queue_cnt, full && !rl, i);
}

#define KC_PROBES 32u
#define KC_EMPTY 0xffffffffu

FDG_DEV uint32_t kc_hash(const uint32_t (&a)[8], uint64_t seed) {
  uint64_t h = seed;
#pragma unroll
  for (int j = 0; j < 4; j++) {
    h ^= ((uint64_t)a[2 * j + 1] << 32) | a[2 * j];
    h *= 0x9e3779b97f4a7c15ull;
    h ^= h >> 29;
  }
  h *= 0xbf58476d1ce4e5b9ull;
  return (uint32_t)(h >> 32) ^ (uint32_t)h;
}

__global__ void __launch_bounds__(256) fdgpu_key_dedup_kernel(const uint8_t *__restrict__ arena,
                                                              const fdgpu_sig_desc_t *__restrict__ sigs,
                                                              uint32_t n_sig_arg, const uint32_t *__restrict__ n_sig_dev,
                                                              uint32_t *__restrict__ ht, uint32_t ht_mask,
                                                              uint32_t *__restrict__ key_of, uint32_t *__restrict__ reps,
                                                              uint32_t *__restrict__ rep_cnt, uint64_t seed) {
  const uint32_t n_sig = n_sig_dev ? *n_sig_dev : n_sig_arg;
  if (blockIdx.x * blockDim.x >= n_sig) return;
  const uint32_t i = blockIdx.x * blockDim.x + threadIdx.x;
  bool is_rep = false;
  if (i < n_sig) {
    uint32_t a[8];
    load32(a, arena + sigs[i].pub_off);
    uint32_t slot = kc_hash(a, seed) & ht_mask, rep = i;
    for (uint32_t p = 0; p < KC_PROBES; p++, slot = (slot + 1u) & ht_mask) {
      uint32_t v = ht[slot];
      if (v == KC_EMPTY) {
        v = atomicCAS(&ht[slot], KC_EMPTY, i);
        if (v == KC_EMPTY) break;
      }
      uint32_t b[8];
      load32(b, arena + sigs[v].pub_off);
      uint32_t diff = 0;
#pragma unroll
      for (int j = 0; j < 8; j++) diff |= a[j] ^ b[j];
      if (!diff) { rep = v; break; }
    }
    key_of[i] = rep;
    is_rep = rep == i;
  }
  __shared__ uint32_t s_cnt, s_base;
  if (threadIdx.x == 0) s_cnt = 0;
  __syncthreads();
  const uint64_t m = __ballot(is_rep);
  const int lane = (int)(threadIdx.x & 63u);
  uint32_t wbase = 0;
  if (m && lane == __ffsll((long long)m) - 1) wbase = atomicAdd(&s_cnt, (uint32_t)__popcll(m));
  if (m) wbase = (uint32_t)__shfl((int)wbase, __ffsll((long long)m) - 1, 64);
  __syncthreads();
  if (threadIdx.x == 0) s_base = s_cnt ? atomicAdd(rep_cnt, s_cnt) : 0u;
  __syncthreads();
  if (is_rep) reps[s_base + wbase + (uint32_t)__popcll(m & ((1ull << lane) - 1ull))] = i;
}

__global__ void __launch_bounds__(FDGPU_BLOCK, FDGPU_VERIFY_WAVES)
fdgpu_key_table_kernel(const uint8_t *__restrict__ arena, const fdgpu_sig_desc_t *__restrict__ sigs,
                       uint32_t *__restrict__ ws, const uint32_t *__restrict__ reps,
                       const uint32_t *__restrict__ rep_cnt, uint32_t *__restrict__ kverd, uint32_t flags) {
  const uint32_t q = blockIdx.x * blockDim.x + threadIdx.x;
  if (q >= *rep_cnt) return;
  const uint32_t i = reps[q];
  uint32_t Aenc[8];
  load32(Aenc, arena + sigs[i].pub_off);
  kverd[i] = decode_neg_table(tab_a(lane_ws(ws, i)), Aenc, (flags & FDGPU_FLAG_REF_MAP) != 0);
}

__global__ void __launch_bounds__(FDGPU_BLOCK, FDGPU_VERIFY_WAVES)
fdgpu_full_kernel(uint32_t *__restrict__ ws, const uint32_t *__restrict__ perm, int8_t *__restrict__ codes,
                  const uint32_t *__restrict__ queue, const uint32_t *__restrict__ queue_cnt, uint32_t slots,
                  const uint32_t *__restrict__ key_of);

FDG_DEV void full_body(uint32_t *__restrict__ ws, const uint32_t *__restrict__ perm, int8_t *__restrict__ codes,
                       const uint32_t *__restrict__ queue, const uint32_t *__restrict__ queue_cnt, uint32_t slots,
                       const uint32_t *__restrict__ key_of, uint32_t bx) {
  const uint32_t cnt = *queue_cnt;
  if (bx * blockDim.x >= cnt) return;
  for (uint32_t q = bx * blockDim.x + threadIdx.x; q < cnt; q += slots) {
    const uint32_t i = queue[q];
    uint32_t *wsl = ws + (size_t)i * FDGPU_WS_LANE_WORDS;
    const uint32_t *park = wsl + FDGPU_WS_PARK * FDGPU_ATAB_WORDS;
    uint32_t kd[KD_WORDS];
#pragma unroll
    for (int j = 0; j < KD_WORDS; j++) kd[j] = park[HPARK_KD + j];
    ge_p2 Rc;
    dsm_k(Rc, kd, wsl, FDGPU_WS_SB, tab_a(key_of ? lane_ws(ws, key_of[i]) : wsl));
    uint32_t er[40];
    atab_load(er, tab_r(wsl), 1);
    fe ypx, ymx, z2, x2, y2, l, r;
#pragma unroll
    for (int j = 0; j < 10; j++) { ypx.v[j] = er[j]; ymx.v[j] = er[10 + j]; z2.v[j] = er[20 + j]; }
    fe_carry(ypx); fe_carry(ymx); fe_carry(z2);
    fe_sub(x2, ymx, ypx);
    fe_add(y2, ypx, ymx);
    fe_mul(l, Rc.X, z2); fe_mul(r, x2, Rc.Z);
    bool eq = fe_eq(l, r);
    fe_mul(l, Rc.Y, z2); fe_mul(r, y2, Rc.Z);
    eq = eq && fe_eq(l, r);
    codes[out_idx(perm, i)] = (int8_t)(eq ? 0 : -3);
  }
}

__global__ void __launch_bounds__(FDGPU_BLOCK, FDGPU_VERIFY_WAVES)
fdgpu_full_kernel(uint32_t *__restrict__ ws, const uint32_t *__restrict__ perm, int8_t *__restrict__ codes,
                  const uint32_t *__restrict__ queue, const uint32_t *__restrict__ queue_cnt, uint32_t slots,
                  const uint32_t *__restrict__ key_of) {
  full_body(ws, perm, codes, queue, queue_cnt, slots, key_of, blockIdx.x);
}

__global__ void __launch_bounds__(FDGPU_BLOCK, FDGPU_VERIFY_WAVES)
fdgpu_full_multi_kernel(const fdgpu_mbatch_t *__restrict__ mb) {
  const fdgpu_mbatch_t b = mb[blockIdx.y];
  if (blockIdx.x >= b.slow) return;
  full_body(b.ws, nullptr, b.codes, b.queue, b.cnt, b.slow * FDGPU_BLOCK, nullptr, blockIdx.x);
}

__global__ void __launch_bounds__(256) fdgpu_combine_kernel(const fdgpu_txn_desc_t *__restrict__ txns, uint32_t n_txn,
                                                            const int8_t *__restrict__ sig_codes,
                                                            int8_t *__restrict__ txn_codes,
                                                            uint64_t *__restrict__ accept) {
  for (uint32_t t0 = blockIdx.x * blockDim.x; t0 < n_txn; t0 += gridDim.x * blockDim.x) {
    const uint32_t t = t0 + threadIdx.x;
    int code = -1;
    if (t < n_txn) {
      const fdgpu_txn_desc_t d = txns[t];
      if (d.sig_cnt >= 1 && d.sig_cnt <= 16) {
        int first_struct = 0, any_msg = 0;
        for (uint32_t j = 0; j < d.sig_cnt; j++) {
          const int c = sig_codes[d.sig0 + j];
          if (c == -3) any_msg = 1;
          else if (c != 0 && first_struct == 0) first_struct = c;
        }
        code = first_struct ? first_struct : (any_msg ? -3 : 0);
      }
      txn_codes[t] = (int8_t)code;
    }
    const uint64_t ok = __ballot(t < n_txn && code == 0);
    if (accept && (threadIdx.x & 63u) == 0 && t < n_txn) accept[t >> 6] = ok;
  }
}

}

extern "C" {

char const *fdgpu_kernel_path(void) { return "halfsize: fdgpu_verify_hs_kernel + fdgpu_full_kernel"; }

int fdgpu_kernel_build_info(char *buf, size_t n) {
  snprintf(buf, n, "\"verify_waves\":%d,\"atab_words\":%u,\"phase_stamps\":%d", (int)FDGPU_VERIFY_WAVES,
           (unsigned)FDGPU_ATAB_WORDS, (int)FDGPU_PHASE_STAMPS);
  return FDGPU_VERIFY_WAVES == 2 && FDGPU_ATAB_WORDS == 40u && FDGPU_PHASE_STAMPS == 0;
}

hipError_t fdgpu_verify_occupancy(int *blocks_per_cu) {
  return hipOccupancyMaxActiveBlocksPerMultiprocessor(blocks_per_cu, fdgpu_verify_hs_kernel<false>, FDGPU_BLOCK, 0);
}

size_t fdgpu_ws_bytes(uint64_t n_sig) { return fdgpu_ws_layout(nullptr, n_sig).bytes; }

hipError_t fdgpu_launch_verify_sigs(const uint8_t *d_arena, const fdgpu_sig_desc_t *d_sigs, uint32_t n_sig,
                                    const uint32_t *d_perm, const uint32_t *d_btab, uint32_t *d_ws,
                                    int8_t *d_sig_codes, uint32_t flags, hipStream_t stream, const uint32_t *d_n_sig,
                                    uint32_t resident_blocks, uint64_t kc_seed, int cnt_zeroed) {
  if (!n_sig) return hipSuccess;
  const uint32_t grid = (n_sig + FDGPU_BLOCK - 1) / FDGPU_BLOCK;
  const fdgpu_ws_layout_t l = fdgpu_ws_layout(d_ws, n_sig);
  hipError_t e = cnt_zeroed ? hipSuccess : hipMemsetAsync(l.cnt, 0, sizeof(uint32_t), stream);
  if (e != hipSuccess) return e;
  if (!resident_blocks) resident_blocks = 1;
  uint32_t slow_blocks = grid < resident_blocks ? grid : resident_blocks;
  const uint32_t slow_cap = grid > 64u ? FDGPU_FULL_BLOCKS : FDGPU_FULL_BLOCKS / 4u;
  if (slow_blocks > slow_cap) slow_blocks = slow_cap;
  const uint32_t *key_of = nullptr;
  if (flags & FDGPU_FLAG_KCACHE) {
    e = hipMemsetAsync(l.ht, 0xff, l.ht_slots * sizeof(uint32_t), stream);
    if (e == hipSuccess) e = hipMemsetAsync(l.rep_cnt, 0, sizeof(uint32_t), stream);
    if (e != hipSuccess) return e;
    hipLaunchKernelGGL(fdgpu_key_dedup_kernel, dim3((n_sig + 255) / 256), dim3(256), 0, stream, d_arena, d_sigs, n_sig,
                       d_n_sig, l.ht, (uint32_t)(l.ht_slots - 1), l.key_of, l.reps, l.rep_cnt, kc_seed);
    hipLaunchKernelGGL(fdgpu_key_table_kernel, dim3(grid), dim3(FDGPU_BLOCK), 0, stream, d_arena, d_sigs, d_ws, l.reps,
                       l.rep_cnt, l.kverd, flags);
    hipLaunchKernelGGL(fdgpu_verify_hs_kernel<true>, dim3(grid), dim3(FDGPU_BLOCK), 0, stream, d_arena, d_sigs, n_sig,
                       d_n_sig, d_btab, d_ws, d_perm, d_sig_codes, l.queue, l.cnt, flags, l.key_of, l.kverd);
    key_of = l.key_of;
  } else if (flags & FDGPU_FLAG_KPAIR) {
    const uint32_t pgrid = (2u * n_sig + FDGPU_BLOCK - 1) / FDGPU_BLOCK;
    hipLaunchKernelGGL(fdgpu_verify_pair_kernel, dim3(pgrid), dim3(FDGPU_BLOCK),
                       (flags & FDGPU_FLAG_KSPREAD) ? FDGPU_SPREAD_LDS_PAIR : 0, stream, d_arena, d_sigs, n_sig,
                       d_n_sig, d_btab, d_ws, d_perm, d_sig_codes, l.queue, l.cnt, flags);
  } else {
    hipLaunchKernelGGL(fdgpu_verify_hs_kernel<false>, dim3(grid), dim3(FDGPU_BLOCK),
                       (flags & FDGPU_FLAG_KSPREAD) ? FDGPU_SPREAD_LDS : 0, stream, d_arena, d_sigs, n_sig,
                       d_n_sig, d_btab, d_ws, d_perm, d_sig_codes, l.queue, l.cnt, flags, nullptr, nullptr);
  }
  hipLaunchKernelGGL(fdgpu_full_kernel, dim3(slow_blocks), dim3(FDGPU_BLOCK), 0, stream, d_ws, d_perm, d_sig_codes,
                     l.queue, l.cnt, slow_blocks * FDGPU_BLOCK, key_of);
  return hipGetLastError();
}

uint64_t fdgpu_sha512_stream_blocks(uint64_t msg_sz) { return (64u + msg_sz + 16u) / 128u + 1u; }

hipError_t fdgpu_launch_sha512_stream(const uint8_t *d_mbuf, uint64_t m0, uint64_t mlen, uint64_t msg_sz,
                                      uint64_t blk0, uint32_t nblk, const uint8_t *d_ra, uint64_t *d_state,
                                      uint32_t n, hipStream_t stream) {
  if (!n || n > 64 || !nblk) return hipErrorInvalidValue;
  hipLaunchKernelGGL(fdgpu_sha512_stream_kernel, dim3(1), dim3(64), 0, stream, d_mbuf, m0, mlen, msg_sz, blk0, nblk,
                     d_ra, d_state, n);
  return hipGetLastError();
}

hipError_t fdgpu_launch_verify_prehashed(const uint8_t *d_arena, const fdgpu_sig_desc_t *d_sigs, uint32_t n_sig,
                                         const uint32_t *d_btab, uint32_t *d_ws, int8_t *d_sig_codes, uint32_t flags,
                                         hipStream_t stream) {
  if (!n_sig) return hipSuccess;
  const uint32_t grid = (n_sig + FDGPU_BLOCK - 1) / FDGPU_BLOCK;
  const fdgpu_ws_layout_t l = fdgpu_ws_layout(d_ws, n_sig);
  hipError_t e = hipMemsetAsync(l.cnt, 0, sizeof(uint32_t), stream);
  if (e != hipSuccess) return e;
  hipLaunchKernelGGL((fdgpu_verify_hs_kernel<false, true>), dim3(grid), dim3(FDGPU_BLOCK), 0, stream, d_arena, d_sigs,
                     n_sig, nullptr, d_btab, d_ws, nullptr, d_sig_codes, l.queue, l.cnt, flags & FDGPU_FLAG_REF_MAP,
                     nullptr, nullptr);
  hipLaunchKernelGGL(fdgpu_full_kernel, dim3(1), dim3(FDGPU_BLOCK), 0, stream, d_ws, nullptr, d_sig_codes, l.queue,
                     l.cnt, FDGPU_BLOCK, nullptr);
  return hipGetLastError();
}

hipError_t fdgpu_launch_verify_multi(const fdgpu_mbatch_t *mb, uint32_t nb, uint32_t grid_max, uint32_t slow_max,
                                     const uint32_t *d_btab, uint32_t flags, hipStream_t stream) {
  if (!nb || !grid_max) return hipSuccess;
  hipLaunchKernelGGL(fdgpu_verify_hs_multi_kernel, dim3(grid_max, nb), dim3(FDGPU_BLOCK), 0, stream, mb, d_btab, flags);
  hipLaunchKernelGGL(fdgpu_full_multi_kernel, dim3(slow_max ? slow_max : 1, nb), dim3(FDGPU_BLOCK), 0, stream, mb);
  return hipGetLastError();
}

hipError_t fdgpu_launch_combine(const fdgpu_txn_desc_t *d_txns, uint32_t n_txn, const int8_t *d_sig_codes,
                                int8_t *d_txn_codes, uint64_t *d_accept, hipStream_t stream) {
  if (!n_txn) return hipSuccess;
  const uint32_t blocks = (n_txn + 255) / 256;
  hipLaunchKernelGGL(fdgpu_combine_kernel, dim3(blocks < FDGPU_AUX_BLOCKS ? blocks : FDGPU_AUX_BLOCKS), dim3(256), 0,
                     stream, d_txns, n_txn, d_sig_codes, d_txn_codes, d_accept);
  return hipGetLastError();
}

#if FDGPU_PHASE_STAMPS
int fdgpu_debug_stamps(uint64_t *out, uint64_t n_waves) {
  if (n_waves > FDGPU_STAMP_WAVES) n_waves = FDGPU_STAMP_WAVES;
  return hipMemcpyFromSymbol(out, HIP_SYMBOL(g_fdgpu_stamps), n_waves * FDGPU_STAMP_SLOTS * sizeof(uint64_t)) ==
                 hipSuccess ? 0 : -1;
}
#endif

}
```

firedancer_amd/ed25519.py:

```python
import ctypes

import numpy as np

from . import _lib

SUCCESS, ERR_SIG, ERR_PUBKEY, ERR_MSG = 0, -1, -2, -3

FLAG_REF_MAPPING = 1
FLAG_NO_BUCKET = 2
FLAG_FULL_PATH = 4
FLAG_KEY_CACHE = 8
FLAG_PAIR = 16
FLAG_PAIR_AUTO = 32
FLAG_MERGE = 64
FLAG_SPREAD = 128
FLAG_SPREAD_AUTO = 256

TXN_DTYPE = np.dtype([("msg_off", "<u4"), ("msg_sz", "<u4"), ("sig_off", "<u4"),
                      ("pub_off", "<u4"), ("sig_cnt", "<u4")])
SIG_DESC_DTYPE = np.dtype([("msg_off", "<u4"), ("msg_sz", "<u4"), ("sig_off", "<u4"), ("pub_off", "<u4")])
TXN_DESC_DTYPE = np.dtype([("sig0", "<u4"), ("sig_cnt", "<u4")])
ARENA_SLACK = 160
SHRED_DTYPE = np.dtype([("off", "<u4"), ("sz", "<u4"), ("pub_off", "<u4")])
CODE_SHRED_REJECT = -67
SHRED_SZ_MAX = 1228 + 4
POH_DTYPE = np.dtype([("hash_cnt", "<u8"), ("prev_off", "<u4"), ("hash_off", "<u4"), ("sig_first", "<u4"),
                      ("sig_cnt", "<u4"), ("mix_off", "<u4"), ("_pad", "<u4")])
POH_NO_MIX = 0xFFFFFFFF
POH_HASH_CNT_MAX = 1 << 20
CODE_POH_MISMATCH = -68
CODE_POH_TOO_LONG = -69


def poh_chunk():
    return int(_lib.lib().fdgpu_poh_chunk())


def bcomb_dims():
    L = _lib.lib()
    return {k: int(L.fdgpu_bcomb_dim(i)) for i, k in enumerate(("w", "ndig", "entries", "stride", "chunk"))}


def ge_ops_shape():
    L = _lib.lib()
    return int(L.fdgpu_test_ge_in_words()), int(L.fdgpu_test_ge_results())


def _poh_arrays(arena, entries, sig_offs):
    return (np.ascontiguousarray(arena, dtype=np.uint8), np.ascontiguousarray(entries, dtype=POH_DTYPE),
            np.ascontiguousarray(sig_offs, dtype=np.uint32))


def verify(msg, sig, public_key, sha=None):
    msg = bytes(msg)
    sig, public_key = bytes(sig), bytes(public_key)
    if len(sig) != 64 or len(public_key) != 32:
        raise ValueError("sig must be 64 bytes and public_key 32 bytes")
    return _lib.lib().fd_ed25519_verify(msg, len(msg), sig, public_key, None)


def verify_batch_single_msg(msg, signatures, pubkeys, shas, batch_sz):
    msg = bytes(msg)
    signatures, pubkeys = bytes(signatures), bytes(pubkeys)
    n = int(batch_sz)
    if n < 0 or n > 255:
        raise ValueError("batch_sz is a uchar")
    if 1 <= n <= 16 and (len(signatures) < 64 * n or len(pubkeys) < 32 * n):
        raise ValueError("signatures/pubkeys shorter than batch_sz records")
    return _lib.lib().fd_ed25519_verify_batch_single_msg(msg, len(msg), signatures, pubkeys, None, n)


def sync_stats():
    import ctypes as c
    v = [c.c_uint64() for _ in range(3)]
    _lib.lib().fdgpu_sync_stats(*[c.byref(x) for x in v])
    return {"calls": v[0].value, "batches": v[1].value, "errors": v[2].value}


def strerror(err):
    return _lib.lib().fd_ed25519_strerror(int(err)).decode()


def expand_txns(txns):
    txns = np.asarray(txns, dtype=TXN_DTYPE)
    cnt = txns["sig_cnt"].astype(np.int64)
    valid = (cnt >= 1) & (cnt <= 16)
    used = np.where(valid, cnt, 0)
    sig0 = np.zeros(len(txns), dtype=np.int64)
    if len(txns):
        sig0[1:] = np.cumsum(used)[:-1]
    n_sig = int(used.sum())
    tdesc = np.zeros(len(txns), dtype=TXN_DESC_DTYPE)
    tdesc["sig0"] = sig0
    tdesc["sig_cnt"] = used
    sdesc = np.zeros(n_sig, dtype=SIG_DESC_DTYPE)
    t_of_sig = np.repeat(np.arange(len(txns)), used)
    j = np.arange(n_sig) - sig0[t_of_sig]
    sdesc["msg_off"] = txns["msg_off"][t_of_sig]
    sdesc["msg_sz"] = txns["msg_sz"][t_of_sig]
    sdesc["sig_off"] = txns["sig_off"][t_of_sig] + 64 * j
    sdesc["pub_off"] = txns["pub_off"][t_of_sig] + 32 * j
    return sdesc, tdesc


class VerifyEngine:

    def __init__(self, device=0, max_txn=1 << 16, max_sig=None, max_arena=None, ring_depth=2, ref_mapping=False,
                 bucket=True, full_path=False, key_cache=False, pair=False, pair_auto=False, merge=False,
                 spread=False, spread_auto=False):
        L = _lib.lib()
        self.max_sig = max_sig or 12 * max_txn
        flags = ((FLAG_REF_MAPPING if ref_mapping else 0) | (0 if bucket else FLAG_NO_BUCKET) |
                 (FLAG_FULL_PATH if full_path else 0) | (FLAG_KEY_CACHE if key_cache else 0) |
                 (FLAG_PAIR if pair else 0) | (FLAG_PAIR_AUTO if pair_auto else 0) | (FLAG_MERGE if merge else 0) |
                 (FLAG_SPREAD if spread else 0) | (FLAG_SPREAD_AUTO if spread_auto else 0))
        cfg = _lib.FdgpuCfg(max_txn, self.max_sig, max_arena or 1232 * max_txn, ring_depth, flags)
        self._cfg = cfg
        self.max_arena = cfg.max_arena
        self._h = L.fdgpu_engine_open(int(device), ctypes.byref(cfg))
        if not self._h:
            raise RuntimeError(f"fdgpu_engine_open({device}) failed: {_lib.last_error()}")
        self.device = device
        self._pending = {}

    def reserve(self, n_sig=0):
        r = _lib.lib().fdgpu_engine_reserve(self._h, int(n_sig))
        if r:
            raise RuntimeError(f"fdgpu_engine_reserve failed: {r} ({_lib.last_error()})")

    def host_register(self, buf):
        arr = np.asarray(buf)
        r = _lib.lib().fdgpu_host_register(self._h, arr.ctypes.data, arr.nbytes)
        if r:
            raise RuntimeError(f"fdgpu_host_register failed: {r} ({_lib.last_error()})")

    def host_unregister(self, buf):
        r = _lib.lib().fdgpu_host_unregister(self._h, np.asarray(buf).ctypes.data)
        if r:
            raise RuntimeError(f"fdgpu_host_unregister failed: {r} ({_lib.last_error()})")

    def close(self):
        if self._h:
            _lib.lib().fdgpu_engine_close(self._h)
            self._h = None

    def __enter__(self):
        return self

    def __exit__(self, *a):
        self.close()

    def __del__(self):
        try:
            self.close()
        except Exception:
            pass

    def info(self):
        g, b, w = ctypes.c_uint32(), ctypes.c_uint32(), ctypes.c_uint64()
        _lib.lib().fdgpu_engine_info(self._h, ctypes.byref(g), ctypes.byref(b), ctypes.byref(w))
        return {"resident_blocks": g.value, "block_threads": b.value, "ws_bytes": w.value}

    def submit(self, arena, txns):
        arena = np.ascontiguousarray(arena, dtype=np.uint8)
        txns = np.ascontiguousarray(txns, dtype=TXN_DTYPE)
        tk = _lib.lib().fdgpu_submit(self._h, arena.ctypes.data, arena.size, txns.ctypes.data, len(txns))
        if tk < 0:
            raise RuntimeError(f"fdgpu_submit failed ({tk}): {_lib.last_error()}")
        self._pending[tk] = len(txns)
        return tk

    def poll(self, ticket, blocking=True):
        n = self._pending.get(ticket)
        if n is None:
            raise KeyError(ticket)
        out = np.zeros(max(n, 1), dtype=np.int8)
        rc = _lib.lib().fdgpu_poll(self._h, ticket, out.ctypes.data, 1 if blocking else 0)
        if rc == 1:
            return None
        if rc != 0:
            raise RuntimeError(f"fdgpu_poll failed ({rc}): {_lib.last_error()}")
        del self._pending[ticket]
        return out[:n]

    def verify_txns(self, arena, txns):
        return self.poll(self.submit(arena, txns), blocking=True)

    def submit_frags(self, arena, frags, trailer_sz):
        arena = np.ascontiguousarray(arena, dtype=np.uint8)
        frags = np.ascontiguousarray(frags, dtype=FRAG_EX_DTYPE)
        tk = _lib.lib().fdgpu_submit_frags(self._h, arena.ctypes.data, arena.size, frags.ctypes.data, len(frags),
                                           int(trailer_sz))
        if tk < 0:
            raise RuntimeError(f"fdgpu_submit_frags failed ({tk}): {_lib.last_error()}")
        self._pending[tk] = (len(frags), int(trailer_sz))
        return tk

    def poll_frags(self, ticket, blocking=True):
        n, tsz = self._pending[ticket]
        codes = np.zeros(max(n, 1), dtype=np.int8)
        tr = np.zeros(max(tsz, 1), dtype=np.uint8)
        rc = _lib.lib().fdgpu_poll_frags(self._h, ticket, codes.ctypes.data, tr.ctypes.data, 1 if blocking else 0)
        if rc == 1:
            return None
        if rc != 0:
            raise RuntimeError(f"fdgpu_poll_frags failed ({rc}): {_lib.last_error()}")
        del self._pending[ticket]
        return codes[:n], tr[:tsz]

    def submit_frags_io(self, frags, out, out_sz, hash_seed, links=None):
        frags = np.ascontiguousarray(frags, dtype=FRAG_IO_DTYPE)
        out = np.asarray(out)
        if out_sz > out.nbytes:
            raise ValueError("out_sz exceeds the out buffer")
        lk = np.array(list(links or []), dtype=LINK_DTYPE)
        tk = _lib.lib().fdgpu_submit_frags_io(self._h, frags.ctypes.data, len(frags), out.ctypes.data, int(out_sz),
                                              int(hash_seed), lk.ctypes.data if len(lk) else None, len(lk))
        if tk < 0:
            raise RuntimeError(f"fdgpu_submit_frags_io failed ({tk}): {_lib.last_error()}")
        self._pending[tk] = (len(frags), frags)
        return tk

    def poll_frags_io(self, ticket, blocking=True):
        n, _ = self._pending[ticket]
        codes = np.zeros(max(n, 1), dtype=np.int8)
        tags = np.zeros(max(n, 1), dtype=np.uint64)
        osz = np.zeros(max(n, 1), dtype=np.uint16)
        rc = _lib.lib().fdgpu_poll_frags_io(self._h, ticket, codes.ctypes.data, tags.ctypes.data, osz.ctypes.data,
                                            1 if blocking else 0)
        if rc == 1:
            return None
        if rc != 0:
            raise RuntimeError(f"fdgpu_poll_frags_io failed ({rc}): {_lib.last_error()}")
        del self._pending[ticket]
        return codes[:n], tags[:n], osz[:n]

    def submit_shreds(self, arena, shreds, expected_version):
        arena = np.ascontiguousarray(arena, dtype=np.uint8)
        shreds = np.ascontiguousarray(shreds, dtype=SHRED_DTYPE)
        tk = _lib.lib().fdgpu_submit_shreds(self._h, arena.ctypes.data, arena.size, shreds.ctypes.data, len(shreds),
                                            int(expected_version))
        if tk < 0:
            raise RuntimeError(f"fdgpu_submit_shreds failed ({tk}): {_lib.last_error()}")
        self._pending[tk] = len(shreds)
        return tk

    def poll_shreds(self, ticket, blocking=True):
        n = self._pending[ticket]
        codes = np.zeros(max(n, 1), dtype=np.int8)
        roots = np.zeros((max(n, 1), 32), dtype=np.uint8)
        rc = _lib.lib().fdgpu_poll_shreds(self._h, ticket, codes.ctypes.data, roots.ctypes.data, 1 if blocking else 0)
        if rc == 1:
            return None
        if rc != 0:
            raise RuntimeError(f"fdgpu_poll_shreds failed ({rc}): {_lib.last_error()}")
        del self._pending[ticket]
        return codes[:n], roots[:n]

    def verify_shreds(self, arena, shreds, expected_version):
        return self.poll_shreds(self.submit_shreds(arena, shreds, expected_version), blocking=True)

    def submit_poh(self, arena, entries, sig_offs, hash_cnt_cap):
        arena, entries, sig_offs = _poh_arrays(arena, entries, sig_offs)
        tk = _lib.lib().fdgpu_submit_poh(self._h, arena.ctypes.data, arena.size, entries.ctypes.data, len(entries),
                                         sig_offs.ctypes.data, len(sig_offs), int(hash_cnt_cap))
        if tk < 0:
            raise RuntimeError(f"fdgpu_submit_poh failed ({tk}): {_lib.last_error()}")
        self._pending[tk] = len(entries)
        return tk

    def poll_poh(self, ticket, blocking=True):
        n = self._pending[ticket]
        codes = np.zeros(max(n, 1), dtype=np.int8)
        hashes = np.zeros((max(n, 1), 32), dtype=np.uint8)
        rc = _lib.lib().fdgpu_poll_poh(self._h, ticket, codes.ctypes.data, hashes.ctypes.data, 1 if blocking else 0)
        if rc == 1:
            return None
        if rc != 0:
            raise RuntimeError(f"fdgpu_poll_poh failed ({rc}): {_lib.last_error()}")
        del self._pending[ticket]
        return codes[:n], hashes[:n]

    def verify_poh(self, arena, entries, sig_offs, hash_cnt_cap):
        return self.poll_poh(self.submit_poh(arena, entries, sig_offs, hash_cnt_cap), blocking=True)

    def verify_device(self, d_arena, d_sig_desc, n_sig, d_txn_desc, n_txn, d_sig_codes, d_txn_codes, stream=0):
        rc = _lib.lib().fdgpu_verify_device(self._h, d_arena, d_sig_desc, n_sig, d_txn_desc, n_txn,
                                            d_sig_codes, d_txn_codes, stream or None)
        if rc != 0:
            raise RuntimeError(f"fdgpu_verify_device failed ({rc}): {_lib.last_error()}")

    def upload(self, arena, txns):
        return DeviceBatch(self, arena, txns)

    def upload_frags(self, arena, frags):
        return FragBatch(self, arena, frags)

    def sync(self):
        self._chk(_lib.lib().fdgpu_sync(self._h), "fdgpu_sync")

    def _chk(self, rc, what):
        if rc != 0:
            raise RuntimeError(f"{what} failed ({rc}): {_lib.last_error()}")

    def debug_fe_ops(self, ab):
        ab = np.ascontiguousarray(ab, dtype=np.uint8).reshape(-1, 64)
        out = np.zeros((len(ab), 8, 32), dtype=np.uint8)
        self._chk(_lib.lib().fdgpu_debug_fe_ops(self._h, ab.ctypes.data, len(ab), out.ctypes.data), "debug_fe_ops")
        return out

    def debug_decode(self, enc, ref_mapping=False):
        enc = np.ascontiguousarray(enc, dtype=np.uint8).reshape(-1, 32)
        out = np.zeros((len(enc), 72), dtype=np.uint8)
        self._chk(_lib.lib().fdgpu_debug_decode(self._h, enc.ctypes.data, len(enc), 1 if ref_mapping else 0,
                                                out.ctypes.data), "debug_decode")
        rc = out[:, 0:4].copy().view(np.int32)[:, 0]
        so = out[:, 4:8].copy().view(np.int32)[:, 0]
        return rc, so, out[:, 8:40], out[:, 40:72]

    def debug_sha512(self, arena, txns):
        arena = np.ascontiguousarray(arena, dtype=np.uint8)
        txns = np.ascontiguousarray(txns, dtype=TXN_DTYPE)
        out = np.zeros((len(txns), 64), dtype=np.uint8)
        self._chk(_lib.lib().fdgpu_debug_sha512(self._h, arena.ctypes.data, arena.size, txns.ctypes.data, len(txns),
                                                out.ctypes.data), "debug_sha512")
        return out

    def debug_sha256(self, arena, txns):
        arena = np.ascontiguousarray(arena, dtype=np.uint8)
        txns = np.ascontiguousarray(txns, dtype=TXN_DTYPE)
        out = np.zeros((len(txns), 32), dtype=np.uint8)
        self._chk(_lib.lib().fdgpu_debug_sha256(self._h, arena.ctypes.data, arena.size, txns.ctypes.data, len(txns),
                                                out.ctypes.data), "debug_sha256")
        return out

    def debug_shred_roots(self, arena, shreds, expected_version):
        arena = np.ascontiguousarray(arena, dtype=np.uint8)
        shreds = np.ascontiguousarray(shreds, dtype=SHRED_DTYPE)
        ok = np.zeros(len(shreds), dtype=np.int8)
        roots = np.zeros((len(shreds), 32), dtype=np.uint8)
        self._chk(_lib.lib().fdgpu_debug_shred_roots(self._h, arena.ctypes.data, arena.size, shreds.ctypes.data,
                                                     len(shreds), int(expected_version), ok.ctypes.data,
                                                     roots.ctypes.data), "debug_shred_roots")
        return ok, roots

    def debug_shred_time(self, arena, shreds, expected_version, iters=5):
        arena = np.ascontiguousarray(arena, dtype=np.uint8)
        shreds = np.ascontiguousarray(shreds, dtype=SHRED_DTYPE)
        a, v = ctypes.c_double(), ctypes.c_double()
        self._chk(_lib.lib().fdgpu_debug_shred_time(self._h, arena.ctypes.data, arena.size, shreds.ctypes.data,
                                                    len(shreds), int(expected_version), int(iters), ctypes.byref(a),
                                                    ctypes.byref(v)), "debug_shred_time")
        return a.value, v.value

    def debug_poh(self, arena, entries, sig_offs, hash_cnt_cap, grid_waves=0):
        arena, entries, sig_offs = _poh_arrays(arena, entries, sig_offs)
        codes = np.zeros(len(entries), dtype=np.int8)
        hashes = np.zeros((len(entries), 32), dtype=np.uint8)
        self._chk(_lib.lib().fdgpu_debug_poh(self._h, arena.ctypes.data, arena.size, entries.ctypes.data, len(entries),
                                             sig_offs.ctypes.data, len(sig_offs), int(hash_cnt_cap), int(grid_waves),
                                             codes.ctypes.data, hashes.ctypes.data), "debug_poh")
        return codes, hashes

    def debug_poh_time(self, arena, entries, sig_offs, hash_cnt_cap, iters=5):
        arena, entries, sig_offs = _poh_arrays(arena, entries, sig_offs)
        t, ch = ctypes.c_double(), ctypes.c_double()
        self._chk(_lib.lib().fdgpu_debug_poh_time(self._h, arena.ctypes.data, arena.size, entries.ctypes.data,
                                                  len(entries), sig_offs.ctypes.data, len(sig_offs), int(hash_cnt_cap),
                                                  int(iters), ctypes.byref(t), ctypes.byref(ch)), "debug_poh_time")
        return t.value, ch.value

    def debug_hram(self, arena, txns):
        arena = np.ascontiguousarray(arena, dtype=np.uint8)
        txns = np.ascontiguousarray(txns, dtype=TXN_DTYPE)
        out = np.zeros((len(txns), 32), dtype=np.uint8)
        self._chk(_lib.lib().fdgpu_debug_hram(self._h, arena.ctypes.data, arena.size, txns.ctypes.data, len(txns),
                                              out.ctypes.data), "debug_hram")
        return out

    def debug_sc_reduce(self, x):
        x = np.ascontiguousarray(x, dtype=np.uint8).reshape(-1, 64)
        out = np.zeros((len(x), 32), dtype=np.uint8)
        self._chk(_lib.lib().fdgpu_debug_sc_reduce(self._h, x.ctypes.data, len(x), out.ctypes.data), "debug_sc_reduce")
        return out

    def debug_hs_split(self, k):
        k = np.ascontiguousarray(k, dtype=np.uint8).reshape(-1, 32)
        out = np.zeros((len(k), 16), dtype=np.uint32)
        self._chk(_lib.lib().fdgpu_debug_hs_split(self._h, k.ctypes.data, len(k), out.ctypes.data), "debug_hs_split")
        return out

    def debug_fe_raw(self, fg):
        fg = np.ascontiguousarray(fg, dtype=np.uint32).reshape(-1, 20)
        out = np.zeros((len(fg), 10, 8), dtype=np.uint32)
        self._chk(_lib.lib().fdgpu_debug_fe_raw(self._h, fg.ctypes.data, len(fg), out.ctypes.data), "debug_fe_raw")
        return out

    def debug_ge_ops(self, rec):
        w_in, n_res = ge_ops_shape()
        rec = np.ascontiguousarray(rec, dtype=np.uint32).reshape(-1, w_in)
        out = np.zeros((len(rec), n_res, 4, 8), dtype=np.uint32)
        self._chk(_lib.lib().fdgpu_debug_ge_ops(self._h, rec.ctypes.data, len(rec), out.ctypes.data), "debug_ge_ops")
        return out

    def debug_sc_recode(self, s):
        s = np.ascontiguousarray(s, dtype=np.uint8).reshape(-1, 32)
        out = np.zeros((len(s), 16), dtype=np.uint32)
        self._chk(_lib.lib().fdgpu_debug_sc_recode(self._h, s.ctypes.data, len(s), out.ctypes.data), "debug_sc_recode")
        return out

    def debug_btab(self):
        d = bcomb_dims()
        out = np.zeros((d["ndig"], d["entries"], d["stride"]), dtype=np.uint32)
        self._chk(_lib.lib().fdgpu_debug_btab(self._h, 0, d["ndig"] * d["entries"], out.ctypes.data), "debug_btab")
        return out

    def debug_sig_codes(self, arena, txns):
        arena = np.ascontiguousarray(arena, dtype=np.uint8)
        txns = np.ascontiguousarray(txns, dtype=TXN_DTYPE)
        cnt = txns["sig_cnt"].astype(np.int64)
        n = int(np.where((cnt >= 1) & (cnt <= 16), cnt, 0).sum())
        out = np.zeros(max(n, 1), dtype=np.int8)
        self._chk(_lib.lib().fdgpu_debug_sig_codes(self._h, arena.ctypes.data, arena.size, txns.ctypes.data,
                                                   len(txns), out.ctypes.data), "debug_sig_codes")
        return out[:n]


class DeviceBatch:

    def __init__(self, engine, arena, txns):
        arena = np.ascontiguousarray(arena, dtype=np.uint8)
        txns = np.ascontiguousarray(txns, dtype=TXN_DTYPE)
        self._e = engine
        self.n_txn = len(txns)
        self._b = _lib.lib().fdgpu_dev_batch_upload(engine._h, arena.ctypes.data, arena.size, txns.ctypes.data,
                                                    len(txns))
        if not self._b:
            raise RuntimeError(f"fdgpu_dev_batch_upload failed: {_lib.last_error()}")
        self.n_sig = int(_lib.lib().fdgpu_dev_batch_sig_cnt(self._b))

    def own_queue(self):
        rc = _lib.lib().fdgpu_dev_batch_own_queue(self._e._h, self._b)
        if rc != 0:
            raise RuntimeError(f"fdgpu_dev_batch_own_queue failed ({rc}): {_lib.last_error()}")
        return self

    def verify(self):
        rc = _lib.lib().fdgpu_dev_batch_verify(self._e._h, self._b)
        if rc != 0:
            raise RuntimeError(f"fdgpu_dev_batch_verify failed ({rc}): {_lib.last_error()}")

    def codes(self, sig_codes=False):
        t = np.zeros(max(self.n_txn, 1), dtype=np.int8)
        s = np.zeros(max(self.n_sig, 1), dtype=np.int8) if sig_codes else None
        rc = _lib.lib().fdgpu_dev_batch_codes(self._e._h, self._b, t.ctypes.data,
                                              s.ctypes.data if s is not None else None)
        if rc != 0:
            raise RuntimeError(f"fdgpu_dev_batch_codes failed ({rc}): {_lib.last_error()}")
        return (t[:self.n_txn], s[:self.n_sig]) if sig_codes else t[:self.n_txn]

    def time(self, iters):
        import ctypes as c
        w, v, k = c.c_double(), c.c_double(), c.c_double()
        rc = _lib.lib().fdgpu_dev_batch_time(self._e._h, self._b, int(iters), c.byref(w), c.byref(v), c.byref(k))
        if rc != 0:
            raise RuntimeError(f"fdgpu_dev_batch_time failed ({rc}): {_lib.last_error()}")
        return w.value, v.value, k.value

    def free(self):
        if self._b:
            _lib.lib().fdgpu_dev_batch_free(self._e._h, self._b)
            self._b = None

    def __del__(self):
        try:
            self.free()
        except Exception:
            pass


FRAG_DTYPE = np.dtype([("off", "<u4"), ("sz", "<u4")])
FRAG_EX_DTYPE = np.dtype([("off", "<u4"), ("sz", "<u4"), ("tr_off", "<u4"), ("tr_cap", "<u4")])
FRAG_IO_DTYPE = np.dtype([("src", "<u8"), ("sz", "<u4"), ("out_off", "<u4"), ("out_cap", "<u4"), ("link", "<u4"),
                          ("seq", "<u8")])
LINK_DTYPE = np.dtype([("mcache", "<u8"), ("depth", "<u8")])
CODE_LAPPED = -66
CODE_TRAILER_CAP = -65
CODE_PARSE_FAIL = -64
TXN_MAX_SZ = 852


class FragBatch(DeviceBatch):

    def __init__(self, engine, arena, frags):
        arena = np.ascontiguousarray(arena, dtype=np.uint8)
        frags = np.ascontiguousarray(frags, dtype=FRAG_DTYPE)
        self._e = engine
        self.n_txn = len(frags)
        self._b = _lib.lib().fdgpu_dev_batch_upload_frags(engine._h, arena.ctypes.data, arena.size,
                                                          frags.ctypes.data, len(frags))
        if not self._b:
            raise RuntimeError(f"fdgpu_dev_batch_upload_frags failed: {_lib.last_error()}")
        sz = frags["sz"].astype(np.int64)
        self.sig_bound = int(np.where(sz >= 134, np.minimum(16, (sz - 38) // 96), 0).sum())
        self.n_sig = self.sig_bound

    def codes(self, sig_codes=False):
        out = super().codes(sig_codes)
        self.n_sig = int(_lib.lib().fdgpu_dev_batch_sig_cnt(self._b))
        if sig_codes:
            return out[0], out[1][:self.n_sig]
        return out

    def txns(self, records=True):
        out = np.zeros((max(self.n_txn, 1), TXN_MAX_SZ), dtype=np.uint8) if records else None
        sz = np.zeros(max(self.n_txn, 1), dtype=np.uint16)
        rc = _lib.lib().fdgpu_dev_batch_txns(self._e._h, self._b, out.ctypes.data if records else None,
                                             sz.ctypes.data)
        if rc != 0:
            raise RuntimeError(f"fdgpu_dev_batch_txns failed ({rc}): {_lib.last_error()}")
        return (out[:self.n_txn] if records else None), sz[:self.n_txn]

    def time2(self, iters):
        import ctypes as c
        w, g, v, k = c.c_double(), c.c_double(), c.c_double(), c.c_double()
        rc = _lib.lib().fdgpu_dev_batch_time2(self._e._h, self._b, int(iters), c.byref(w), c.byref(g), c.byref(v),
                                              c.byref(k))
        if rc != 0:
            raise RuntimeError(f"fdgpu_dev_batch_time2 failed ({rc}): {_lib.last_error()}")
        return w.value, g.value, v.value, k.value
```

Before: 108.5 million sigs/s.

## Pack per-lane point tables into 32-word entries and split aux workspace

Table entries for the A and R precomputed points are tightened and packed from 40 limb words into 32 words, with the top limbs bit-packed into the spare high bits of the lower limbs. The SB point and park data move to a separate auxiliary region addressed downward from the queue pointer. This cuts global memory traffic and LDS staging size per table lookup, and the LDS budget for the spread kernels is rederived so one block fits per CU. In exchange, every load and store now does extra carry, pack and unpack ALU work, and there is a new debug kernel for testing the packing.

```diff
diff --git a/firedancer_amd/_lib.py b/firedancer_amd/_lib.py
--- a/firedancer_amd/_lib.py
+++ b/firedancer_amd/_lib.py
@@ -156,6 +156,7 @@
     L.fdgpu_debug_ge_ops.argtypes = [vp, vp, c.c_uint64, vp]
     L.fdgpu_debug_sc_recode.argtypes = [vp, vp, c.c_uint64, vp]
     L.fdgpu_debug_btab.argtypes = [vp, c.c_uint64, c.c_uint64, vp]
+    L.fdgpu_debug_tabpack.argtypes = [vp, vp, c.c_uint64, vp]
     L.fdgpu_bcomb_dim.argtypes = [c.c_int]
     L.fdgpu_bcomb_dim.restype = c.c_uint32
     L.fdgpu_test_ge_in_words.argtypes = []
@@ -164,7 +165,8 @@
     L.fdgpu_test_ge_results.restype = c.c_uint32
     for fn in ("fdgpu_debug_fe_ops", "fdgpu_debug_decode", "fdgpu_debug_sha512", "fdgpu_debug_hram",
                "fdgpu_debug_sc_reduce", "fdgpu_debug_hs_split", "fdgpu_debug_sig_codes",
-               "fdgpu_debug_fe_raw", "fdgpu_debug_ge_ops", "fdgpu_debug_sc_recode", "fdgpu_debug_btab"):
+               "fdgpu_debug_fe_raw", "fdgpu_debug_ge_ops", "fdgpu_debug_sc_recode", "fdgpu_debug_btab",
+               "fdgpu_debug_tabpack"):
         getattr(L, fn).restype = c.c_int
     _LIB = L
     return L
diff --git a/firedancer_amd/csrc/fdgpu_atab.h b/firedancer_amd/csrc/fdgpu_atab.h
--- /dev/null
+++ b/firedancer_amd/csrc/fdgpu_atab.h
@@ -0,0 +1,136 @@
+#pragma once
+
+#include <hip/hip_runtime.h>
+
+#include "fdgpu_ge.h"
+#include "fdgpu_internal.h"
+
+namespace fdgpu {
+
+FDG_DEV void fe_tight(fe &h) {
+#pragma unroll
+  for (int pass = 0; pass < 2; pass++) {
+#pragma unroll
+    for (int i = 0; i < 9; i++) {
+      const int w = (i & 1) ? 25 : 26;
+      h.v[i + 1] += h.v[i] >> w;
+      h.v[i] &= (1u << w) - 1;
+    }
+    const uint32_t c = h.v[9] >> 25;
+    h.v[9] &= (1u << 25) - 1;
+    h.v[0] += 19u * c;
+  }
+}
+
+FDG_DEV void fe_pack8(uint32_t (&w)[8], const fe &t) {
+#pragma unroll
+  for (int h = 0; h < 2; h++) {
+    const uint32_t s = t.v[8 + h];
+    w[4 * h + 0] = t.v[4 * h + 0] | (s << 26);
+    w[4 * h + 1] = t.v[4 * h + 1] | ((s >> 6) << 25);
+    w[4 * h + 2] = t.v[4 * h + 2] | ((s >> 13) << 26);
+    w[4 * h + 3] = t.v[4 * h + 3] | ((s >> 19) << 25);
+  }
+}
+
+FDG_DEV void fe_unpack8(uint32_t *q, const uint32_t (&w)[8]) {
+#pragma unroll
+  for (int j = 0; j < 8; j++) q[j] = w[j] & ((j & 1) ? (1u << 25) - 1 : (1u << 26) - 1);
+#pragma unroll
+  for (int h = 0; h < 2; h++) {
+    uint32_t s = w[4 * h + 3] >> 25;
+    s = (s << 6) | (w[4 * h + 2] >> 26);
+    s = (s << 7) | (w[4 * h + 1] >> 25);
+    s = (s << 6) | (w[4 * h + 0] >> 26);
+    q[8 + h] = s;
+  }
+}
+
+__host__ __device__ constexpr int atab_pos(int c, int j) {
+  return c >= 2 ? 8 * c + j : 4 * (j / 2) + 2 * c + (j % 2);
+}
+
+struct alignas(128) tab_ident_t { uint32_t w[FDGPU_PTAB_WORDS]; };
+static __device__ const tab_ident_t g_tab_ident = {{1u, 0u, 1u, 0u, 0u, 0u, 0u, 0u, 0u, 0u, 0u, 0u, 0u, 0u, 0u, 0u, 2u}};
+static_assert(atab_pos(0, 0) == 0 && atab_pos(1, 0) == 2 && atab_pos(2, 0) == 16 && atab_pos(3, 7) == 31 &&
+              atab_pos(0, 7) == 13 && atab_pos(1, 7) == 15, "the stored order (and the identity entry's)");
+
+FDG_DEV const uint32_t *tab_entry(const uint32_t *tab, int e) {
+  return e ? tab + (uint32_t)(e < 0 ? -e : e) * FDGPU_PTAB_WORDS : g_tab_ident.w;
+}
+
+FDG_DEV void atab_store(uint32_t *tab, uint32_t entry, const ge_cached &c) {
+  uint4 *p = (uint4 *)(tab + entry * FDGPU_PTAB_WORDS);
+  uint32_t o[FDGPU_PTAB_WORDS];
+#pragma unroll
+  for (int cc = 0; cc < 4; cc++) {
+    fe t = cc == 0 ? c.YpX : cc == 1 ? c.YmX : cc == 2 ? c.Z2 : c.T2d;
+    fe_tight(t);
+    uint32_t w[8];
+    fe_pack8(w, t);
+#pragma unroll
+    for (int j = 0; j < 8; j++) o[atab_pos(cc, j)] = w[j];
+  }
+#pragma unroll
+  for (int q = 0; q < 8; q++) p[q] = make_uint4(o[4 * q], o[4 * q + 1], o[4 * q + 2], o[4 * q + 3]);
+}
+
+FDG_DEV void atab_unpack(uint32_t (&q)[40], const uint32_t (&o)[FDGPU_PTAB_WORDS]) {
+#pragma unroll
+  for (int cc = 0; cc < 4; cc++) {
+    uint32_t w[8];
+#pragma unroll
+    for (int j = 0; j < 8; j++) w[j] = o[atab_pos(cc, j)];
+    fe_unpack8(q + 10 * cc, w);
+  }
+}
+
+FDG_DEV void atab_load(uint32_t (&q)[40], const uint32_t *tab, int e) {
+  const uint4 *ent = (const uint4 *)tab_entry(tab, e);
+  uint32_t o[FDGPU_PTAB_WORDS];
+#pragma unroll
+  for (int i = 0; i < 8; i++) {
+    const uint4 v = ent[i];
+    o[4 * i] = v.x; o[4 * i + 1] = v.y; o[4 * i + 2] = v.z; o[4 * i + 3] = v.w;
+  }
+  atab_unpack(q, o);
+}
+
+FDG_DEV uint32_t atab_limb(const uint32_t *ent, int c, int w) {
+  if (w < 8) return ent[atab_pos(c, w)] & ((w & 1) ? (1u << 25) - 1 : (1u << 26) - 1);
+  const int b = 4 * (w - 8);
+  uint32_t s = ent[atab_pos(c, b + 3)] >> 25;
+  s = (s << 6) | (ent[atab_pos(c, b + 2)] >> 26);
+  s = (s << 7) | (ent[atab_pos(c, b + 1)] >> 25);
+  s = (s << 6) | (ent[atab_pos(c, b + 0)] >> 26);
+  return s;
+}
+
+typedef __attribute__((address_space(3))) void lds_void_t;
+
+FDG_DEV void stage_entry(uint32_t *lds_wave, const uint32_t *tab, int e) {
+  const uint32_t *src = tab_entry(tab, e);
+  constexpr int NCH = FDGPU_PTAB_WORDS / 4;
+#pragma unroll
+  for (int c = 0; c < NCH; c++)
+    __builtin_amdgcn_global_load_lds((const void *)(src + 4 * c), (lds_void_t *)(lds_wave + 256 * c), 16, 0, 0);
+}
+
+FDG_DEV void unstage_entry_signed(uint32_t (&q)[40], const uint32_t *lds_wave, bool neg) {
+  const uint32_t lane = threadIdx.x & 63u;
+  const uint32_t *a = lds_wave + 4 * lane + (neg ? 2u : 0u), *b = lds_wave + 4 * lane + (neg ? 0u : 2u);
+  uint32_t o[FDGPU_PTAB_WORDS];
+#pragma unroll
+  for (int c = 0; c < 4; c++) {
+    const uint2 x = *(const uint2 *)(a + 256 * c), y = *(const uint2 *)(b + 256 * c);
+    o[4 * c] = x.x; o[4 * c + 1] = x.y; o[4 * c + 2] = y.x; o[4 * c + 3] = y.y;
+  }
+#pragma unroll
+  for (int c = 4; c < 8; c++) {
+    const uint4 v = *(const uint4 *)(lds_wave + 256 * c + 4 * lane);
+    o[4 * c] = v.x; o[4 * c + 1] = v.y; o[4 * c + 2] = v.z; o[4 * c + 3] = v.w;
+  }
+  atab_unpack(q, o);
+}
+
+}
diff --git a/firedancer_amd/csrc/fdgpu_diag.cpp b/firedancer_amd/csrc/fdgpu_diag.cpp
--- a/firedancer_amd/csrc/fdgpu_diag.cpp
+++ b/firedancer_amd/csrc/fdgpu_diag.cpp
@@ -94,6 +94,10 @@
   return debug_map(e, s, n, 8, 16, out, fdgpu_launch_test_sc_recode);
 }
 
+int fdgpu_debug_tabpack(fdgpu_engine_t *e, uint8_t const *in, uint64_t n, uint8_t *out) {
+  return debug_map(e, in, n, FDGPU_ATAB_WORDS, FDGPU_TABPACK_OUT_WORDS, out, fdgpu_launch_test_tabpack);
+}
+
 int fdgpu_debug_btab(fdgpu_engine_t *e, uint64_t first_entry, uint64_t n_entries, uint32_t *out) {
   const uint64_t total = (uint64_t)FDGPU_BCOMB_NDIG * FDGPU_BCOMB_ENTRIES;
   if (!e || !e->d_btab || !out || first_entry > total || n_entries > total - first_entry) {
diff --git a/firedancer_amd/csrc/fdgpu_internal.h b/firedancer_amd/csrc/fdgpu_internal.h
--- a/firedancer_amd/csrc/fdgpu_internal.h
+++ b/firedancer_amd/csrc/fdgpu_internal.h
@@ -24,6 +24,7 @@
 #ifndef FDGPU_ATAB_WORDS
 #define FDGPU_ATAB_WORDS    40u
 #endif
+#define FDGPU_PTAB_WORDS    32u
 #ifndef FDGPU_VERIFY_WAVES
 #define FDGPU_VERIFY_WAVES  2
 #endif
@@ -38,18 +39,30 @@
 #define HS_MAX_WIN          40u
 #define FDGPU_TAB_STORED    (FDGPU_ATAB_ENTRIES - 1u)
 #define FDGPU_WS_RTAB       FDGPU_TAB_STORED
-#define FDGPU_WS_PARK       (2u * FDGPU_TAB_STORED)
-#define FDGPU_WS_SB         (FDGPU_WS_PARK + 1u)
-#define FDGPU_WS_ENTRIES    (FDGPU_WS_SB + 1u)
+#define FDGPU_WS_ENTRIES    (2u * FDGPU_TAB_STORED + 2u)
 #define FDGPU_WS_LANE_WORDS (FDGPU_WS_ENTRIES * FDGPU_ATAB_WORDS)
+#define FDGPU_WS_TAB_WORDS  (2u * FDGPU_TAB_STORED * FDGPU_PTAB_WORDS)
+#define FDGPU_WS_AUX_WORDS  (FDGPU_WS_LANE_WORDS - FDGPU_WS_TAB_WORDS)
+#define FDGPU_AUX_PARK      0u
+#define FDGPU_AUX_SB        FDGPU_ATAB_WORDS
 #define FDGPU_BLOCK         256u
 #define FDGPU_FLAG_REF_MAP  1u
 #define FDGPU_FLAG_KFULL    2u
 #define FDGPU_FLAG_KCACHE   4u
 #define FDGPU_FLAG_KPAIR    8u
 #define FDGPU_FLAG_KSPREAD  16u
-#define FDGPU_SPREAD_LDS       1024u
-#define FDGPU_SPREAD_LDS_PAIR  (40u * 1024u + 1024u)
+#define FDGPU_STAGE_WAVE_WORDS (FDGPU_PTAB_WORDS / 4u * 256u)
+#define FDGPU_STAGE_LDS        (FDGPU_BLOCK / 64u * 2u * FDGPU_STAGE_WAVE_WORDS * 4u)
+#define FDGPU_STAGE_LDS_PAIR   (FDGPU_BLOCK / 64u * FDGPU_STAGE_WAVE_WORDS * 4u)
+#define FDGPU_CU_LDS           (160u * 1024u)
+#define FDGPU_SPREAD_LDS       (FDGPU_CU_LDS / 2u - FDGPU_STAGE_LDS + 1024u)
+#define FDGPU_SPREAD_LDS_PAIR  (FDGPU_CU_LDS / 2u - FDGPU_STAGE_LDS_PAIR + 1024u)
+#ifdef __cplusplus
+static_assert(2u * (FDGPU_STAGE_LDS + FDGPU_SPREAD_LDS) > FDGPU_CU_LDS &&
+              2u * (FDGPU_STAGE_LDS_PAIR + FDGPU_SPREAD_LDS_PAIR) > FDGPU_CU_LDS &&
+              FDGPU_STAGE_LDS + FDGPU_SPREAD_LDS <= FDGPU_CU_LDS && FDGPU_STAGE_LDS_PAIR + FDGPU_SPREAD_LDS_PAIR <= FDGPU_CU_LDS,
+              "a spread launch's LDS admits one block per CU, and no more");
+#endif
 #define FDGPU_FULL_BLOCKS   16u
 #define FDGPU_AUX_BLOCKS    64u
 #define FDGPU_IO_BLOCKS     16u
@@ -164,10 +177,13 @@
 uint32_t   fdgpu_test_ge_results(void);
 hipError_t fdgpu_launch_test_ge(const uint32_t *d_in, uint32_t *d_out, uint32_t n, hipStream_t stream);
 hipError_t fdgpu_launch_test_sc_recode(const uint32_t *d_in, uint32_t *d_out, uint32_t n, hipStream_t stream);
+#define FDGPU_TABPACK_OUT_WORDS 160u
+hipError_t fdgpu_launch_test_tabpack(const uint32_t *d_in, uint32_t *d_out, uint32_t n, hipStream_t stream);
 
 int      fdgpu_debug_fe_raw(fdgpu_engine_t *e, uint8_t const *fg, uint64_t n, uint8_t *out);
 int      fdgpu_debug_ge_ops(fdgpu_engine_t *e, uint8_t const *in, uint64_t n, uint8_t *out);
 int      fdgpu_debug_sc_recode(fdgpu_engine_t *e, uint8_t const *s, uint64_t n, uint8_t *out);
+int      fdgpu_debug_tabpack(fdgpu_engine_t *e, uint8_t const *in, uint64_t n, uint8_t *out);
 int      fdgpu_debug_btab(fdgpu_engine_t *e, uint64_t first_entry, uint64_t n_entries, uint32_t *out);
 uint32_t fdgpu_bcomb_dim(int which);
 
diff --git a/firedancer_amd/csrc/fdgpu_test_kernels.hip b/firedancer_amd/csrc/fdgpu_test_kernels.hip
--- a/firedancer_amd/csrc/fdgpu_test_kernels.hip
+++ b/firedancer_amd/csrc/fdgpu_test_kernels.hip
@@ -1,5 +1,6 @@
 #include <hip/hip_runtime.h>
 
+#include "fdgpu_atab.h"
 #include "fdgpu_ge.h"
 #include "fdgpu_hram.h"
 #include "fdgpu_internal.h"
@@ -229,6 +230,32 @@
   for (int j = 0; j < 8; j++) { w[j] = d16[j]; w[8 + j] = j < NW ? dc[j] : 0u; }
 }
 
+__global__ void __launch_bounds__(64) fdgpu_test_tabpack_kernel(const uint32_t *in, uint32_t *out, uint32_t n) {
+  __shared__ uint32_t s_stage[FDGPU_STAGE_WAVE_WORDS];
+  const uint32_t i = blockIdx.x * blockDim.x + threadIdx.x;
+  if (i >= n) return;
+  const uint32_t *src = in + FDGPU_ATAB_WORDS * (size_t)i;
+  uint32_t *dst = out + FDGPU_TABPACK_OUT_WORDS * (size_t)i;
+  ge_cached c;
+#pragma unroll
+  for (int w = 0; w < 10; w++) { c.YpX.v[w] = src[w]; c.YmX.v[w] = src[10 + w]; c.Z2.v[w] = src[20 + w]; c.T2d.v[w] = src[30 + w]; }
+  uint32_t *tab = dst - FDGPU_PTAB_WORDS;
+  atab_store(tab, 1, c);
+  __threadfence();
+  uint32_t q[40];
+  atab_load(q, tab, 1);
+#pragma unroll
+  for (int w = 0; w < 40; w++) dst[32 + w] = q[w];
+  stage_entry(s_stage, tab, 1);
+  asm volatile("s_waitcnt vmcnt(0)" ::: "memory");
+  unstage_entry_signed(q, s_stage, false);
+#pragma unroll
+  for (int w = 0; w < 40; w++) dst[72 + w] = q[w];
+  unstage_entry_signed(q, s_stage, true);
+#pragma unroll
+  for (int w = 0; w < 40; w++) dst[112 + w] = q[w];
+}
+
 }
 
 extern "C" {
@@ -274,5 +301,9 @@
   hipLaunchKernelGGL(fdgpu_test_sc_recode_kernel, dim3((n + 63) / 64), dim3(64), 0, stream, d_in, d_out, n);
   return hipGetLastError();
 }
-
-}
+hipError_t fdgpu_launch_test_tabpack(const uint32_t *d_in, uint32_t *d_out, uint32_t n, hipStream_t stream) {
+  hipLaunchKernelGGL(fdgpu_test_tabpack_kernel, dim3((n + 63) / 64), dim3(64), 0, stream, d_in, d_out, n);
+  return hipGetLastError();
+}
+
+}
diff --git a/firedancer_amd/csrc/fdgpu_verify.hip b/firedancer_amd/csrc/fdgpu_verify.hip
--- a/firedancer_amd/csrc/fdgpu_verify.hip
+++ b/firedancer_amd/csrc/fdgpu_verify.hip
@@ -1,5 +1,6 @@
 #include <hip/hip_runtime.h>
 
+#include "fdgpu_atab.h"
 #include "fdgpu_bcomb.h"
 #include "fdgpu_ge.h"
 #include "fdgpu_hram.h"
@@ -14,46 +15,29 @@
 namespace {
 
 
-__host__ __device__ constexpr int atab_pos(int w) {
-  return w >= 20 ? w : w < 10 ? 4 * (w / 2) + (w % 2) : 4 * ((w - 10) / 2) + 2 + (w % 2);
-}
-
-struct alignas(16) tab_ident_t { uint32_t w[FDGPU_ATAB_WORDS]; };
-__device__ const tab_ident_t g_tab_ident = {{1u, 0u, 1u, 0u, 0u, 0u, 0u, 0u, 0u, 0u, 0u, 0u, 0u, 0u, 0u, 0u, 0u, 0u, 0u, 0u, 2u}};
-static_assert(atab_pos(0) == 0 && atab_pos(10) == 2 && atab_pos(20) == 20, "identity entry's stored order");
-
-FDG_DEV const uint32_t *tab_entry(const uint32_t *tab, int e) {
-  return e ? tab + (uint32_t)(e < 0 ? -e : e) * FDGPU_ATAB_WORDS : g_tab_ident.w;
-}
-FDG_DEV uint32_t *tab_a(uint32_t *wsl) { return wsl - FDGPU_ATAB_WORDS; }
-FDG_DEV const uint32_t *tab_a(const uint32_t *wsl) { return wsl - FDGPU_ATAB_WORDS; }
-FDG_DEV uint32_t *tab_r(uint32_t *wsl) { return wsl + (FDGPU_WS_RTAB - 1u) * FDGPU_ATAB_WORDS; }
-
-FDG_DEV void atab_store(uint32_t *wsl, uint32_t entry, const ge_cached &c) {
-  uint4 *p = (uint4 *)(wsl + entry * FDGPU_ATAB_WORDS);
-  uint32_t w[40], o[40];
+FDG_DEV uint32_t *tab_a(uint32_t *wsl) { return wsl - FDGPU_PTAB_WORDS; }
+FDG_DEV const uint32_t *tab_a(const uint32_t *wsl) { return wsl - FDGPU_PTAB_WORDS; }
+FDG_DEV uint32_t *tab_r(uint32_t *wsl) { return wsl + (FDGPU_WS_RTAB - 1u) * FDGPU_PTAB_WORDS; }
+
+FDG_DEV void sb_store(uint32_t *aux, const ge_cached &c) {
+  uint4 *p = (uint4 *)(aux + FDGPU_AUX_SB);
+  uint32_t w[40];
 #pragma unroll
   for (int i = 0; i < 10; i++) { w[i] = c.YpX.v[i]; w[10 + i] = c.YmX.v[i]; w[20 + i] = c.Z2.v[i]; w[30 + i] = c.T2d.v[i]; }
 #pragma unroll
-  for (int i = 0; i < 40; i++) o[atab_pos(i)] = w[i];
-#pragma unroll
-  for (int q = 0; q < 10; q++) p[q] = make_uint4(o[4 * q], o[4 * q + 1], o[4 * q + 2], o[4 * q + 3]);
-}
-FDG_DEV int sext4(uint32_t x) { return ((int)(x << 28)) >> 28; }
-
-#define KD_WORDS 8
-
-FDG_DEV void atab_load(uint32_t (&q)[40], const uint32_t *wsl, int e) {
-  const uint4 *ent = (const uint4 *)tab_entry(wsl, e);
-  uint32_t o[40];
+  for (int q = 0; q < 10; q++) p[q] = make_uint4(w[4 * q], w[4 * q + 1], w[4 * q + 2], w[4 * q + 3]);
+}
+FDG_DEV void sb_load(uint32_t (&q)[40], const uint32_t *aux) {
+  const uint4 *ent = (const uint4 *)(aux + FDGPU_AUX_SB);
 #pragma unroll
   for (int i = 0; i < 10; i++) {
     const uint4 v = ent[i];
-    o[4 * i] = v.x; o[4 * i + 1] = v.y; o[4 * i + 2] = v.z; o[4 * i + 3] = v.w;
-  }
-#pragma unroll
-  for (int i = 0; i < 40; i++) q[i] = o[atab_pos(i)];
-}
+    q[4 * i] = v.x; q[4 * i + 1] = v.y; q[4 * i + 2] = v.z; q[4 * i + 3] = v.w;
+  }
+}
+FDG_DEV int sext4(uint32_t x) { return ((int)(x << 28)) >> 28; }
+
+#define KD_WORDS 8
 
 FDG_DEV void shl4(uint32_t (&w)[8]) {
 #pragma unroll
@@ -61,9 +45,7 @@
   w[0] <<= 4;
 }
 
-FDG_DEV void dsm_k(ge_p2 &acc2, uint32_t (&kd)[KD_WORDS], const uint32_t *wsl, uint32_t sb_entry = FDGPU_WS_SB,
-                   const uint32_t *ta = nullptr) {
-  if (!ta) ta = tab_a(wsl);
+FDG_DEV void dsm_k(ge_p2 &acc2, uint32_t (&kd)[KD_WORDS], const uint32_t *aux, const uint32_t *ta) {
   ge_p3 acc3;
   ge_p1p1 t;
   uint32_t q[40];
@@ -90,7 +72,7 @@
   }
   ge_p1p1_to_p3(acc3, t);
   uint32_t qs[40];
-  atab_load(qs, wsl, (int)sb_entry);
+  sb_load(qs, aux);
   ge_add_cached_regs(t, acc3, qs, false);
   ge_p1p1_to_p2(acc2, t);
 }
@@ -147,8 +129,8 @@
   ge_p1p1 t; ge_p2 a2; ge_p3 P;
   ge_p3_to_p2(a2, An); ge_dbl(t, a2); ge_p1p1_to_p3(P, t);
   ge_p3_to_cached(c, P); atab_store(wsl, 2, c);
-  const uint32_t *ent1 = wsl + 1u * FDGPU_ATAB_WORDS;
-  auto ld1 = [ent1](int cc, int w) { return ent1[atab_pos(10 * cc + w)]; };
+  const uint32_t *ent1 = wsl + 1u * FDGPU_PTAB_WORDS;
+  auto ld1 = [ent1](int cc, int w) { return atab_limb(ent1, cc, w); };
 #pragma unroll 1
   for (uint32_t e = 3; e < FDGPU_ATAB_ENTRIES; e++) {
     if (e & 1u) {
@@ -165,7 +147,13 @@
 }
 
 FDG_DEV uint32_t *lane_ws(uint32_t *ws, uint32_t i) {
-  return ws + (size_t)i * FDGPU_WS_LANE_WORDS;
+  return ws + (size_t)i * FDGPU_WS_TAB_WORDS;
+}
+FDG_DEV uint32_t *lane_aux(uint32_t *queue, uint32_t i) {
+  return queue - ((size_t)i + 1u) * FDGPU_WS_AUX_WORDS;
+}
+FDG_DEV const uint32_t *lane_aux(const uint32_t *queue, uint32_t i) {
+  return queue - ((size_t)i + 1u) * FDGPU_WS_AUX_WORDS;
 }
 
 FDG_DEV uint32_t out_idx(const uint32_t *__restrict__ perm, uint32_t i) { return perm ? perm[i] : i; }
@@ -173,7 +161,9 @@
 
 #define HPARK_KD 0
 #define HPARK_CODE 30
-static_assert(HPARK_KD + KD_WORDS <= HPARK_CODE && HPARK_CODE < (int)FDGPU_ATAB_WORDS, "park layout");
+static_assert(HPARK_KD + KD_WORDS <= HPARK_CODE && HPARK_CODE < (int)FDGPU_AUX_SB - (int)FDGPU_AUX_PARK &&
+              FDGPU_AUX_SB + FDGPU_ATAB_WORDS <= FDGPU_WS_AUX_WORDS && FDGPU_AUX_SB % 4u == 0 && FDGPU_WS_AUX_WORDS % 4u == 0,
+              "aux layout");
 
 FDG_DEV void recode16_160(uint32_t (&out)[5], uint32_t &nd, const uint32_t (&m)[5]) {
   uint32_t carry = 0;
@@ -231,35 +221,11 @@
   }
 }
 
-typedef __attribute__((address_space(3))) void lds_void_t;
-
-FDG_DEV void stage_entry(uint32_t *lds_wave, const uint32_t *tab, int e) {
-  const uint32_t *src = tab_entry(tab, e);
-  constexpr int NCH = 10;
-#pragma unroll
-  for (int c = 0; c < NCH; c++)
-    __builtin_amdgcn_global_load_lds((const void *)(src + 4 * c), (lds_void_t *)(lds_wave + 256 * c), 16, 0, 0);
-}
-
-FDG_DEV void unstage_entry_signed(uint32_t (&q)[40], const uint32_t *lds_wave, bool neg) {
-  const uint32_t lane = threadIdx.x & 63u;
-  const uint32_t *a = lds_wave + 4 * lane + (neg ? 2u : 0u), *b = lds_wave + 4 * lane + (neg ? 0u : 2u);
-#pragma unroll
-  for (int c = 0; c < 5; c++) {
-    const uint2 x = *(const uint2 *)(a + 256 * c), y = *(const uint2 *)(b + 256 * c);
-    q[2 * c] = x.x; q[2 * c + 1] = x.y; q[10 + 2 * c] = y.x; q[10 + 2 * c + 1] = y.y;
-  }
-#pragma unroll
-  for (int c = 5; c < 10; c++) {
-    const uint4 v = *(const uint4 *)(lds_wave + 256 * c + 4 * lane);
-    q[4 * c] = v.x; q[4 * c + 1] = v.y; q[4 * c + 2] = v.z; q[4 * c + 3] = v.w;
-  }
-}
-
 FDG_DEV void hs_chain(ge_p1p1 &t, uint32_t (&ud)[5], uint32_t (&vd)[5], bool u_neg, bool v_neg, uint32_t nwin,
                       const uint32_t *wsl, const uint32_t *ta) {
   const uint32_t *tr = tab_r(const_cast<uint32_t *>(wsl));
-  __shared__ uint32_t s_stage[FDGPU_BLOCK / 64][2][10 * 256];
+  __shared__ uint32_t s_stage[FDGPU_BLOCK / 64][2][FDGPU_STAGE_WAVE_WORDS];
+  static_assert(sizeof(s_stage) == FDGPU_STAGE_LDS, "FDGPU_SPREAD_LDS is derived from this");
   uint32_t *st_r = &s_stage[threadIdx.x >> 6][0][0];
   uint32_t *st_a = &s_stage[threadIdx.x >> 6][1][0];
   ge_p2 acc2;
@@ -363,7 +329,7 @@
 #pragma unroll
   for (int off = 32; off > 0; off >>= 1) nb = max(nb, (uint32_t)__shfl_xor((int)nb, off));
   uint32_t *wsl = lane_ws(ws, i);
-  uint32_t *park = wsl + FDGPU_WS_PARK * FDGPU_ATAB_WORDS;
+  uint32_t *aux = lane_aux(queue, i);
   const uint32_t *ta = tab_a(wsl);
   FDGPU_STAMP(0);
   uint32_t Renc[8], Aenc[8];
@@ -429,9 +395,9 @@
     ge_p3 WB;
     comb_sb(WB, w, btab);
     ge_cached c; ge_p3_to_cached(c, WB);
-    atab_store(wsl, FDGPU_WS_SB, c);
-  }
-  if (full) park_full(park, k);
+    sb_store(aux, c);
+  }
+  if (full) park_full(aux + FDGPU_AUX_PARK, k);
   FDGPU_STAMP(6);
   bool eq = false;
   if (__any(half)) {
@@ -441,7 +407,7 @@
     ge_p1p1 t;
     hs_chain(t, ud, vd, hs.u_neg, hs.v_neg, nwin, wsl, ta);
     uint32_t q[40];
-    atab_load(q, wsl, (int)FDGPU_WS_SB);
+    sb_load(q, aux);
     fe ypx, ymx, z2, xw, yw, l1, l2;
 #pragma unroll
     for (int j = 0; j < 10; j++) { ypx.v[j] = q[j]; ymx.v[j] = q[10 + j]; z2.v[j] = q[20 + j]; }
@@ -517,7 +483,8 @@
 
 
 FDG_DEV void hs_chain1(ge_p1p1 &t, uint32_t (&dd)[5], bool neg, uint32_t nwin, const uint32_t *tab) {
-  __shared__ uint32_t s_stage1[FDGPU_BLOCK / 64][10 * 256];
+  __shared__ uint32_t s_stage1[FDGPU_BLOCK / 64][FDGPU_STAGE_WAVE_WORDS];
+  static_assert(sizeof(s_stage1) == FDGPU_STAGE_LDS_PAIR, "FDGPU_SPREAD_LDS_PAIR is derived from this");
   uint32_t *st = &s_stage1[threadIdx.x >> 6][0];
   ge_p2 acc2;
   ge_p3 acc3;
@@ -566,6 +533,7 @@
   const fdgpu_sig_desc_t d = sigs[active ? i : n_sig - 1];
   const uint32_t nb = wave_max_u32(sha512_hram_blocks(d.msg_sz));
   uint32_t *wsl = lane_ws(ws, i);
+  uint32_t *aux = lane_aux(queue, i);
   uint32_t *tab = rl ? tab_r(wsl) : tab_a(wsl);
   uint32_t Renc[8], Aenc[8];
   load32(Renc, arena + d.sig_off);
@@ -609,9 +577,9 @@
     ge_p1p1 tw; ge_add_cached(tw, WB, c, false);
     ge_p1p1_to_p3(WB, tw);
     ge_p3_to_cached(c, WB);
-    if (!rl) atab_store(wsl, FDGPU_WS_SB, c);
-  }
-  if (full && !rl) park_full(wsl + FDGPU_WS_PARK * FDGPU_ATAB_WORDS, k);
+    if (!rl) sb_store(aux, c);
+  }
+  if (full && !rl) park_full(aux + FDGPU_AUX_PARK, k);
   bool eq = false;
   if (__any(half)) {
     const uint32_t nwin = wave_max_u32(half ? nd_lane : 1u);
@@ -632,7 +600,7 @@
     ge_p3_to_cached(oc, other);
     ge_add_cached(t, mine, oc, false);
     uint32_t q[40];
-    atab_load(q, wsl, (int)FDGPU_WS_SB);
+    sb_load(q, aux);
     fe ypx, ymx, z2, xw, yw, l1, l2;
 #pragma unroll
     for (int j = 0; j < 10; j++) { ypx.v[j] = q[j]; ymx.v[j] = q[10 + j]; z2.v[j] = q[20 + j]; }
@@ -734,13 +702,13 @@
   if (bx * blockDim.x >= cnt) return;
   for (uint32_t q = bx * blockDim.x + threadIdx.x; q < cnt; q += slots) {
     const uint32_t i = queue[q];
-    uint32_t *wsl = ws + (size_t)i * FDGPU_WS_LANE_WORDS;
-    const uint32_t *park = wsl + FDGPU_WS_PARK * FDGPU_ATAB_WORDS;
+    uint32_t *wsl = lane_ws(ws, i);
+    const uint32_t *aux = lane_aux(queue, i), *park = aux + FDGPU_AUX_PARK;
     uint32_t kd[KD_WORDS];
 #pragma unroll
     for (int j = 0; j < KD_WORDS; j++) kd[j] = park[HPARK_KD + j];
     ge_p2 Rc;
-    dsm_k(Rc, kd, wsl, FDGPU_WS_SB, tab_a(key_of ? lane_ws(ws, key_of[i]) : wsl));
+    dsm_k(Rc, kd, aux, tab_a(key_of ? lane_ws(ws, key_of[i]) : wsl));
     uint32_t er[40];
     atab_load(er, tab_r(wsl), 1);
     fe ypx, ymx, z2, x2, y2, l, r;
diff --git a/firedancer_amd/ed25519.py b/firedancer_amd/ed25519.py
--- a/firedancer_amd/ed25519.py
+++ b/firedancer_amd/ed25519.py
@@ -409,6 +409,12 @@
         self._chk(_lib.lib().fdgpu_debug_sc_recode(self._h, s.ctypes.data, len(s), out.ctypes.data), "debug_sc_recode")
         return out
 
+    def debug_tabpack(self, ent):
+        ent = np.ascontiguousarray(ent, dtype=np.uint32).reshape(-1, 40)
+        out = np.zeros((len(ent), 160), dtype=np.uint32)
+        self._chk(_lib.lib().fdgpu_debug_tabpack(self._h, ent.ctypes.data, len(ent), out.ctypes.data), "debug_tabpack")
+        return out[:, :32].copy(), out[:, 32:152].reshape(-1, 3, 40).copy()
+
     def debug_btab(self):
         d = bcomb_dims()
         out = np.zeros((d["ndig"], d["entries"], d["stride"]), dtype=np.uint32)
```

Result: faster. 110.5 million sigs/s (median of 6 runs) (+1.8%).
